# spacejam/loghisto

Hardware: NVIDIA H100
Metric: histogram ingest throughput (samples/s) (higher is better)
Workload: dtype f64

## Files before the change

### loghisto_b200/csrc/lh_api.cu

```cuda
#include "../../include/loghisto_b200.h"
#include "lh_kernels.cuh"

#include <algorithm>
#include <cmath>
#include <condition_variable>
#include <cstdio>
#include <cstring>
#include <mutex>
#include <new>
#include <string>
#include <vector>
#include <unistd.h>

using namespace lh;

namespace {

struct WriterEvent { cudaStream_t stream; cudaEvent_t ev; };

struct Buffer {
    unsigned long long *d_buckets = nullptr;
    unsigned long long *d_counters = nullptr;
    uint32_t *d_flags = nullptr;
    unsigned int *d_hot = nullptr;
    unsigned long long hot_pending = 0;
    cudaEvent_t cleared = nullptr;
    std::vector<WriterEvent> writers;
};

enum SlotState { SLOT_FREE = 0, SLOT_ACQUIRED = 1 , SLOT_INFLIGHT = 2,
                 SLOT_WAITED = 3 ,
                 SLOT_FILLING = 4  };
struct Slot {
    void *h = nullptr; void *d = nullptr;
    cudaEvent_t done = nullptr;
    cudaEvent_t copied = nullptr;
    int state = SLOT_FREE;
    uint64_t seq = 0;
};

struct K1Variant {
    const char *name;
    void (*launch)(int grid, size_t smem, cudaStream_t s, const double *v32, size_t nvec,
                   const double *head, int nhead, const double *tail, int ntail, unsigned long long *counts,
                   uint32_t *flag, const Prec &pc);
    const void *func;
    int threads;
    size_t smem_fixed;
    int blocks_per_sm;
    size_t smem;
};

template <int THREADS, int UNROLL, int MINB>
void launch_ldg(int grid, size_t smem, cudaStream_t s, const double *v32, size_t nvec, const double *head, int nhead,
                const double *tail, int ntail, unsigned long long *counts, uint32_t *flag, const Prec &pc) {
    k_ingest_single_ldg<THREADS, UNROLL, MINB><<<grid, THREADS, smem, s>>>(v32, nvec, head, nhead, tail, ntail, counts, flag, pc);
}
template <int CW, int STAGES, int STAGE_BYTES, int MINB, bool FOLD>
void launch_bulk(int grid, size_t smem, cudaStream_t s, const double *v32, size_t nvec, const double *head, int nhead,
                 const double *tail, int ntail, unsigned long long *counts, uint32_t *flag, const Prec &pc) {
    k_ingest_single_bulk<CW, STAGES, STAGE_BYTES, MINB, FOLD><<<grid, (CW + 1) * 32, smem, s>>>(v32, nvec, head, nhead, tail, ntail, counts, flag, pc);
}
void launch_probe(int grid, size_t, cudaStream_t s, const double *v32, size_t nvec, const double *head, int nhead,
                  const double *tail, int ntail, unsigned long long *counts, uint32_t *flag, const Prec &pc) {
    k_stream_probe<512, 4><<<grid, 512, 0, s>>>(v32, nvec, head, nhead, tail, ntail, counts, flag, pc);
}

#define LDG_VARIANT(T, U, M) \
    { "ldg_t" #T "_u" #U "_b" #M, launch_ldg<T, U, M>, (const void *)k_ingest_single_ldg<T, U, M>, T, 0, 0, 0 }
#define BULK_VARIANT(W, S, B, M, F) \
    { "bulk2_w" #W "_s" #S "_" #B "_b" #M "_sign" #F, launch_bulk<W, S, B, M, F != 0>, (const void *)k_ingest_single_bulk<W, S, B, M, F != 0>, (W + 1) * 32, \
      (size_t)S * B + (size_t)S * 16, 0, 0 }

K1Variant g_k1_variants[] = {
    BULK_VARIANT(16, 4, 32768, 1, 1),
    BULK_VARIANT(16, 3, 65536, 1, 1),
    BULK_VARIANT(8, 4, 16384, 2, 1),
    LDG_VARIANT(512, 2, 2),
    { "probe_read_only_t512_u4", launch_probe, (const void *)k_stream_probe<512, 4>, 512, 0, 0, 0 },
    BULK_VARIANT(16, 4, 32768, 1, 0),
    BULK_VARIANT(16, 3, 65536, 1, 0),
};
constexpr int kNumK1Variants = (int)(sizeof(g_k1_variants) / sizeof(g_k1_variants[0]));
constexpr int kDefaultK1Variant = 6;

Prec make_prec(uint32_t precision) {
    Prec pc{};
    const double P = (double)precision;
    const double c1 = P * 0.6931471805599453094172321;
    pc.precision = P;
    pc.a_int = (uint32_t)std::floor(c1);
    pc.c1 = (float)c1;
    pc.c2 = (float)(c1 - (double)pc.a_int);
    pc.kb = (float)(-1023.0 * (double)pc.c2);
    const float eps = 0.000244140625f * (precision > 100 ? (float)P / 100.0f : 1.0f);
    pc.thresh = 0.5f - eps;
    pc.win = (uint32_t)std::floor(P * 63.0 * 0.6931471805599453094172321 + 0.5) + 1u;
    pc.a4 = pc.a_int * 4u;
    pc.coff = 0u - 1023u * pc.a4 - (0x4B400000u << 2);
    pc.coff0 = 0u - 1023u * pc.a_int - 0x4B400000u;
    return pc;
}

constexpr int kMaxRanks = LH_MAX_RANKS;
constexpr int kCommWords = 2 * LH_MAX_RANKS;
constexpr uint32_t kPeerMagic = 0x4C485052u;

struct PeerWire {
    uint32_t magic, abi, H, C;
    uint32_t precision, device;
    int64_t pid;
    uint64_t ctx_id;
    uint64_t ptr_buckets[2], ptr_flags[2], ptr_counters[2], ptr_comm, ptr_red;
    cudaIpcMemHandle_t ipc_buckets[2], ipc_flags[2], ipc_counters[2], ipc_comm, ipc_red;
};
static_assert(sizeof(PeerWire) <= LH_PEER_HANDLE_BYTES, "lh_peer_handle too small");

struct PeerMap {
    unsigned long long *buckets[2] = {nullptr, nullptr};
    uint32_t *flags[2] = {nullptr, nullptr};
    unsigned long long *counters[2] = {nullptr, nullptr};
    unsigned long long *comm = nullptr;
    unsigned long long *red = nullptr;
    bool ipc = false;
};

}

struct lh_ctx {
    lh_config cfg{};
    int device = 0;
    int sm_count = 0;
    uint32_t H = 0, C = 0;
    Prec pc{};
    Buffer buf[2];
    int active = 0;
    bool frozen = false;
    bool nnz_valid = false;
    cudaStream_t ingest_stream = nullptr, snap_stream = nullptr, copy_stream = nullptr;
    double *d_decomp = nullptr;
    unsigned long long *d_dropped = nullptr;
    double *d_ps[3] = {nullptr, nullptr, nullptr};
    char *d_res[3] = {nullptr, nullptr, nullptr};
    char *h_res[3] = {nullptr, nullptr, nullptr};
    cudaEvent_t res_done[3] = {nullptr, nullptr, nullptr};
    uint32_t res_np[3] = {0, 0, 0};
    uint64_t res_ticket[2] = {0, 0};
    uint64_t next_ticket = 1;
    uint32_t *d_nnz = nullptr, *d_offsets = nullptr;
    short *d_x_keys = nullptr; unsigned long long *d_x_counts = nullptr; size_t x_cap = 0;
    uint32_t *h_offsets = nullptr;
    short *h_x_keys = nullptr; unsigned long long *h_x_counts = nullptr; size_t hx_cap = 0;
    unsigned long long *h_counter_deltas = nullptr;
    std::vector<Slot> slots;
    uint64_t slot_seq = 0;
    size_t staging_bytes = 0;
    unsigned long long last_margin[2] = {0, 0};
    int k1_variant = kDefaultK1Variant;
    int k1_grid_mult = 1;
    int k1_reserve_sms = 0;
    int keyed_blocks_per_sm = 8;
    uint32_t hot_replicas = 1;
    int keyed_mode = 0;
    int64_t kp_chunk = 256 << 20;
    uint32_t wc_pf_tiles = 1;
    uint32_t wc_flush_samples = 24576;
    int wc_spt = 6;
    unsigned short *d_kp_queues = nullptr;
    unsigned int *d_kp_cnt = nullptr;
    uint4 *d_kp_rare = nullptr;
    size_t kp_cap = 0;
    int kp_parts = 0;
    const char *keyed_kernel = "";
    uint32_t comm_rank = 0, comm_world = 0;
    unsigned long long *d_comm = nullptr;
    unsigned int *d_comm_aux = nullptr;
    PeerMap peers[kMaxRanks];
    unsigned long long *d_red_buckets = nullptr;
    uint32_t *d_red_flags = nullptr;
    unsigned long long *d_red_counters = nullptr;
    bool view_reduced = false;
    bool view_counters_reduced = false;
    uint64_t comm_seq = 0;
    bool comm_two_shot = false;
    static constexpr int kCommRing = 8;
    cudaEvent_t comm_t0[kCommRing] = {}, comm_t1[kCommRing] = {};
    uint64_t ctx_id = 0;
    std::mutex rs_mu;
    cudaStream_t rs_stream = nullptr;
    unsigned long long *d_rs_rows = nullptr;
    uint32_t *d_rs_flags = nullptr, *d_rs_nnz = nullptr;
    bool rs_dirty = false;
    K1Variant k1[kNumK1Variants];
    static constexpr int kTimingRing = 16;
    cudaEvent_t ev_t0s[kTimingRing] = {}, ev_t1s[kTimingRing] = {};
    cudaEvent_t ev_t0 = nullptr, ev_t1 = nullptr;
    uint64_t ingest_seq = 0;
    bool timing_valid = false;
    lh_stats stats{};
    std::mutex mu;
    std::condition_variable slot_cv;
    std::string last_error;
};

namespace {

lh_status fail(lh_ctx *ctx, lh_status st, const char *what, cudaError_t e = cudaSuccess) {
    if (ctx) {
        char buf[512];
        if (e != cudaSuccess) snprintf(buf, sizeof buf, "%s: %s (%s)", what, cudaGetErrorName(e), cudaGetErrorString(e));
        else snprintf(buf, sizeof buf, "%s", what);
        ctx->last_error = buf;
    }
    return st;
}

#define LH_CUDA(ctx, call)                                                      \
    do {                                                                        \
        cudaError_t _e = (call);                                                \
        if (_e != cudaSuccess) return fail((ctx), LH_ERR_CUDA, #call, _e);      \
    } while (0)

lh_status before_write(lh_ctx *ctx, int b, cudaStream_t s) {
    LH_CUDA(ctx, cudaStreamWaitEvent(s, ctx->buf[b].cleared, 0));
    return LH_OK;
}
lh_status after_write(lh_ctx *ctx, int b, cudaStream_t s) {
    for (auto &w : ctx->buf[b].writers)
        if (w.stream == s) { LH_CUDA(ctx, cudaEventRecord(w.ev, s)); return LH_OK; }
    WriterEvent w{s, nullptr};
    LH_CUDA(ctx, cudaEventCreateWithFlags(&w.ev, cudaEventDisableTiming));
    LH_CUDA(ctx, cudaEventRecord(w.ev, s));
    ctx->buf[b].writers.push_back(w);
    return LH_OK;
}

void next_timing_slot(lh_ctx *ctx) {
    const int i = (int)(ctx->ingest_seq % lh_ctx::kTimingRing);
    ctx->ev_t0 = ctx->ev_t0s[i];
    ctx->ev_t1 = ctx->ev_t1s[i];
    ctx->ingest_seq++;
}

cudaStream_t pick_stream(lh_ctx *ctx, void *stream) { return stream ? (cudaStream_t)stream : ctx->ingest_stream; }

int grid_1d(lh_ctx *ctx, size_t n, int threads, int per_thread, int blocks_per_sm) {
    size_t need = (n + (size_t)threads * per_thread - 1) / ((size_t)threads * per_thread);
    size_t cap = (size_t)ctx->sm_count * blocks_per_sm;
    return (int)std::max<size_t>(1, std::min(need, cap));
}

lh_status launch_single(lh_ctx *ctx, uint32_t hid, const double *d_values, size_t n, cudaStream_t s) {
    if (hid >= ctx->H) return fail(ctx, LH_ERR_RANGE, "histogram_id >= max_histograms");
    if (((uintptr_t)d_values & 7u) != 0) return fail(ctx, LH_ERR_INVALID, "d_values must be 8-byte aligned");
    const int b = ctx->active;
    lh_status st = before_write(ctx, b, s);
    if (st != LH_OK) return st;
    unsigned long long *counts = ctx->buf[b].d_buckets + (size_t)hid * 65536u;
    uint32_t *flag = ctx->buf[b].d_flags + hid;
    const K1Variant &kv = ctx->k1[ctx->k1_variant];
    const int grid = std::max(1, ctx->sm_count - ctx->k1_reserve_sms) * kv.blocks_per_sm * ctx->k1_grid_mult;
    const size_t kMaxPerLaunch = std::min((size_t)1 << 36, (size_t)grid << 31);
    size_t done = 0;
    next_timing_slot(ctx);
    LH_CUDA(ctx, cudaEventRecord(ctx->ev_t0, s));
    while (done < n) {
        size_t m = std::min(n - done, kMaxPerLaunch);
        const double *p = d_values + done;
        int nhead = (int)(((32u - ((uintptr_t)p & 31u)) & 31u) / 8u);
        if ((size_t)nhead > m) nhead = (int)m;
        const double *head = p;
        const double *body = p + nhead;
        size_t nvec = (m - nhead) >> 2;
        const double *tail = body + nvec * 4;
        int ntail = (int)(m - nhead - nvec * 4);
        kv.launch(grid, kv.smem, s, body, nvec, head, nhead, tail, ntail, counts, flag, ctx->pc);
        LH_CUDA(ctx, cudaGetLastError());
        ctx->stats.kernel_launches++;
        done += m;
    }
    LH_CUDA(ctx, cudaEventRecord(ctx->ev_t1, s));
    ctx->timing_valid = true;
    ctx->stats.samples += n;
    return after_write(ctx, b, s);
}

lh_status fold_hot(lh_ctx *ctx, int b, cudaStream_t s) {
    const size_t cells = (size_t)ctx->H * 2u * ctx->pc.win;
    int grid = (int)std::min<size_t>((cells + 255) / 256, (size_t)ctx->sm_count * 16);
    k_fold_hot<<<grid, 256, 0, s>>>(ctx->buf[b].d_hot, ctx->buf[b].d_buckets, ctx->buf[b].d_flags, cells, ctx->hot_replicas, ctx->pc.win);
    LH_CUDA(ctx, cudaGetLastError());
    ctx->stats.kernel_launches++;
    ctx->buf[b].hot_pending = 0;
    return LH_OK;
}

KeyedOut keyed_out(lh_ctx *ctx, int b) {
    KeyedOut o{};
    o.hot = ctx->buf[b].d_hot; o.buckets = ctx->buf[b].d_buckets; o.flags = ctx->buf[b].d_flags;
    o.dropped = ctx->d_dropped; o.H = ctx->H;
    return o;
}

uint32_t ks_ids_per_pass(const lh_ctx *ctx) { return std::max<uint32_t>(1, (uint32_t)(KS_SMEM_BYTES / ((size_t)ctx->pc.win * 4))); }

constexpr size_t kSmemBudget = 227 * 1024;
template <typename IdT, typename ValT, int SPT>
lh_status launch_keyed_wc_spt(lh_ctx *ctx, int b, const IdT *ids, const ValT *vals, size_t n4x4, cudaStream_t s, bool *used, size_t *taken,
                              const IdT *ids2 = nullptr, const long long *vals2 = nullptr, size_t n2 = 0, size_t *taken2 = nullptr) {
    *used = false;
    *taken = 0;
    if (taken2) *taken2 = 0;
    const int P = std::min(ctx->sm_count - ctx->k1_reserve_sms, (int)WC_MAX_PARTS);
    if (P < 8 || n4x4 + n2 == 0) return LH_OK;
    const uint32_t ids_per = (ctx->H + P - 1) / P;
    using S = WcShape<SPT>;
    const size_t hist_bytes = (((size_t)ids_per * ctx->pc.win + 3) & ~(size_t)3) * 4;
    uint32_t row_cap = 0;
    size_t smem = 0;
    for (uint32_t cap_try : {256u, 192u, 128u}) {
        smem = hist_bytes + 2 * WC_MAX_PARTS * 4 + (size_t)(P + 1) * (cap_try + WC_ROW_EXTRA) * 2;
        if (smem <= kSmemBudget) { row_cap = cap_try; break; }
    }
    if (!row_cap || (size_t)ids_per * ctx->pc.win > 65535) return LH_OK;
    if (ctx->keyed_mode != 2 && n4x4 + n2 < ((size_t)1 << 22)) return LH_OK;
    n4x4 = n4x4 / S::TILE * S::TILE;
    n2 = n2 / S::TILE * S::TILE;
    if (n4x4 + n2 == 0) return LH_OK;
    const size_t slice_max = std::max<size_t>(1, ((size_t)ctx->kp_chunk + (size_t)P * S::TILE - 1) / ((size_t)P * S::TILE));
    const size_t tiles_all = n4x4 / S::TILE + n2 / S::TILE;
    const size_t nchunks = (tiles_all + slice_max * P - 1) / (slice_max * P);
    const size_t slice_tiles = std::max<size_t>(1, (tiles_all + nchunks * P - 1) / (nchunks * P));
    const size_t expect = slice_max * S::TILE / P;
    const size_t cap = ((expect * 5 / 4 + 3 * WC_LINE + WC_LINE - 1) / WC_LINE) * WC_LINE;
    if (!ctx->d_kp_queues || ctx->kp_cap != cap || ctx->kp_parts != P) {
        cudaFree(ctx->d_kp_queues); cudaFree(ctx->d_kp_cnt); cudaFree(ctx->d_kp_rare);
        ctx->d_kp_queues = nullptr; ctx->d_kp_cnt = nullptr; ctx->d_kp_rare = nullptr;
        LH_CUDA(ctx, cudaMalloc(&ctx->d_kp_rare, (size_t)P * WC_RARE_CAP * sizeof(uint4)));
        LH_CUDA(ctx, cudaMalloc(&ctx->d_kp_queues, (size_t)2 * P * P * cap * sizeof(unsigned short)));
        LH_CUDA(ctx, cudaMalloc(&ctx->d_kp_cnt, ((size_t)2 * P * P + 1) * sizeof(unsigned int)));
        ctx->kp_cap = cap; ctx->kp_parts = P;
    }
    const void *fn = (const void *)k_ingest_keyed_wc<IdT, ValT, SPT, false>;
    if constexpr (std::is_same<ValT, double>::value) {
        if (n2) fn = (const void *)k_ingest_keyed_wc<IdT, double, SPT, true>;
    }
    LH_CUDA(ctx, cudaFuncSetAttribute(fn, cudaFuncAttributeMaxDynamicSharedMemorySize, (int)smem));
    unsigned int *d_barrier = ctx->d_kp_cnt + (size_t)2 * P * P;
    LH_CUDA(ctx, cudaMemsetAsync(d_barrier, 0, sizeof(unsigned int), s));
    WcParams prm{};
    prm.ids = ids; prm.vals = vals; prm.n = n4x4; prm.ids_per = ids_per; prm.cap = (uint32_t)cap;
    prm.ids2 = ids2; prm.vals2 = vals2; prm.n2 = n2;
    prm.inv_p = (uint32_t)(((uint64_t)1 << 32) / (uint64_t)P) + 1u;
    const double room = (double)row_cap - 63.0;
    const double m_max = std::pow((-3.5 + std::sqrt(3.5 * 3.5 + 4.0 * room)) / 2.0, 2.0);
    const uint32_t flush_samples = std::min<uint32_t>(ctx->wc_flush_samples, (uint32_t)(m_max * P));
    prm.flush_tiles = std::max<uint32_t>(1u, flush_samples / S::TILE);
    prm.pf_tiles = ctx->wc_pf_tiles;
    prm.row_cap = row_cap;
    prm.row_stride = row_cap + WC_ROW_EXTRA;
    prm.slice_tiles = (uint32_t)slice_tiles; prm.queues = ctx->d_kp_queues; prm.q_cnt = ctx->d_kp_cnt;
    prm.barrier = d_barrier; prm.rare = ctx->d_kp_rare; prm.o = keyed_out(ctx, b);
    Prec pc = ctx->pc;
    void *args[] = {&prm, &pc};
    LH_CUDA(ctx, cudaLaunchCooperativeKernel(fn, dim3(P), dim3(S::THREADS), args, smem, s));
    ctx->stats.kernel_launches++;
    *used = true;
    *taken = n4x4;
    if (taken2) *taken2 = n2;
    return LH_OK;
}
template <typename IdT, typename ValT>
lh_status launch_keyed_wc(lh_ctx *ctx, int b, const IdT *ids, const ValT *vals, size_t n4x4, cudaStream_t s, bool *used, size_t *taken,
                          const IdT *ids2 = nullptr, const long long *vals2 = nullptr, size_t n2 = 0, size_t *taken2 = nullptr) {
#define LH_WC_SHAPE(code) case code: return launch_keyed_wc_spt<IdT, ValT, code>(ctx, b, ids, vals, n4x4, s, used, taken, ids2, vals2, n2, taken2);
    switch (ctx->wc_spt) {
        LH_WC_SHAPE(6) LH_WC_SHAPE(4) LH_WC_SHAPE(3)
        default: return launch_keyed_wc_spt<IdT, ValT, 8>(ctx, b, ids, vals, n4x4, s, used, taken, ids2, vals2, n2, taken2);
    }
#undef LH_WC_SHAPE
}

template <typename IdT, typename ValT>
lh_status launch_keyed(lh_ctx *ctx, const IdT *d_ids, const ValT *d_vals, size_t n, cudaStream_t s) {
    if (((uintptr_t)d_vals & 7u) || ((uintptr_t)d_ids & (sizeof(IdT) - 1)))
        return fail(ctx, LH_ERR_INVALID, "ids / values are not naturally aligned");
    const int b = ctx->active;
    lh_status st = before_write(ctx, b, s);
    if (st != LH_OK) return st;
    constexpr int T = 256;
    const KeyedOut ko = keyed_out(ctx, b);
    next_timing_slot(ctx);
    LH_CUDA(ctx, cudaEventRecord(ctx->ev_t0, s));
    size_t done = 0;
    while (done < n) {
        const unsigned long long kCap = 0xFFFFFFFFull;
        if (ctx->buf[b].hot_pending >= kCap - (1ull << 30)) { st = fold_hot(ctx, b, s); if (st != LH_OK) return st; }
        size_t m = (size_t)std::min<unsigned long long>(n - done, kCap - ctx->buf[b].hot_pending);
        const IdT *ids = d_ids + done;
        const ValT *vals = d_vals + done;
        size_t head = std::min<size_t>(m, ((32u - ((uintptr_t)vals & 31u)) & 31u) / 8u);
        bool vec_ok = (((uintptr_t)(ids + head)) & (4 * sizeof(IdT) - 1)) == 0;
        size_t n4 = vec_ok ? (m - head) / 4 : 0;
        size_t tail_off = head + n4 * 4;
        if (!vec_ok) { head = 0; tail_off = 0; }
        if (head) {
            k_ingest_keyed<IdT, ValT, T><<<1, T, 0, s>>>(ids, vals, head, ko, ctx->pc);
            ctx->stats.kernel_launches++;
        }
        size_t hot_used = 0;
        if (n4) {
            bool used = false;
            constexpr uint32_t KS_MAX_PASSES = 4;
            const uint32_t per_max = ks_ids_per_pass(ctx);
            const uint32_t passes = (ctx->H + per_max - 1) / per_max;
            if (passes <= KS_MAX_PASSES && ctx->keyed_mode == 0 && n4 >= 4096) {
                const uint32_t per = (ctx->H + passes - 1) / passes;
                const size_t smem = ((size_t)per * ctx->pc.win + 4) * 4;
                const void *fn = (const void *)k_ingest_keyed_small<IdT, ValT>;
                LH_CUDA(ctx, cudaFuncSetAttribute(fn, cudaFuncAttributeMaxDynamicSharedMemorySize, (int)smem));
                int grid = (int)std::max<size_t>(1, std::min<size_t>((size_t)(ctx->sm_count - ctx->k1_reserve_sms),
                                                                      n4 / (KS_THREADS * 16)));
                for (uint32_t lo = 0; lo < ctx->H; lo += per) {
                    const uint32_t cnt = std::min(per, ctx->H - lo);
                    k_ingest_keyed_small<IdT, ValT><<<grid, KS_THREADS, smem, s>>>(ids + head, vals + head, n4, lo, cnt, ko, ctx->pc);
                    ctx->stats.kernel_launches++;
                }
                used = true;
                hot_used = n4 * 4;
                ctx->keyed_kernel = "k_ingest_keyed_small";
            }
            if (!used && ctx->keyed_mode != 1) {
                size_t taken = 0;
                st = launch_keyed_wc<IdT, ValT>(ctx, b, ids + head, vals + head, n4 * 4, s, &used, &taken);
                if (st != LH_OK) return st;
                if (used) {
                    ctx->keyed_kernel = "k_ingest_keyed_wc";
                    tail_off = head + taken;
                }
            }
            if (!used) {
                int grid = grid_1d(ctx, n4, T, 1, ctx->keyed_blocks_per_sm);
                k_ingest_keyed_vec<IdT, ValT, T><<<grid, T, 0, s>>>(ids + head, vals + head, n4, ctx->hot_replicas, ko, ctx->pc);
                ctx->stats.kernel_launches++;
                hot_used = n4 * 4;
                ctx->keyed_kernel = "k_ingest_keyed_vec";
            }
        }
        if (tail_off < m) {
            size_t r = m - tail_off;
            int grid = grid_1d(ctx, r, T, 1, ctx->keyed_blocks_per_sm);
            k_ingest_keyed<IdT, ValT, T><<<grid, T, 0, s>>>(ids + tail_off, vals + tail_off, r, ko, ctx->pc);
            ctx->stats.kernel_launches++;
        }
        LH_CUDA(ctx, cudaGetLastError());
        ctx->buf[b].hot_pending += hot_used;
        done += m;
    }
    LH_CUDA(ctx, cudaEventRecord(ctx->ev_t1, s));
    ctx->timing_valid = true;
    ctx->stats.samples += n;
    return after_write(ctx, b, s);
}

template <typename IdT>
lh_status launch_keyed_pair(lh_ctx *ctx, const IdT *ids_f, const double *vals_f, size_t n_f, const IdT *ids_ns, const long long *vals_ns,
                            size_t n_ns, cudaStream_t s) {
    auto aligned = [](const void *v, const void *i) { return (((uintptr_t)v & 31u) == 0) && (((uintptr_t)i & (4 * sizeof(IdT) - 1)) == 0); };
    const uint32_t small_passes = (ctx->H + ks_ids_per_pass(ctx) - 1) / ks_ids_per_pass(ctx);
    const bool small = small_passes <= 4 && ctx->keyed_mode == 0;
    const bool fuse = n_f && n_ns && ctx->keyed_mode != 1 && !small && aligned(vals_f, ids_f) && aligned(vals_ns, ids_ns);
    if (fuse) {
        const int b = ctx->active;
        lh_status st = before_write(ctx, b, s);
        if (st != LH_OK) return st;
        next_timing_slot(ctx);
        LH_CUDA(ctx, cudaEventRecord(ctx->ev_t0, s));
        bool used = false;
        size_t took_f = 0, took_ns = 0;
        st = launch_keyed_wc<IdT, double>(ctx, b, ids_f, vals_f, n_f, s, &used, &took_f, ids_ns, vals_ns, n_ns, &took_ns);
        if (st != LH_OK) return st;
        if (used) {
            constexpr int T = 256;
            const KeyedOut ko = keyed_out(ctx, b);
            ctx->keyed_kernel = "k_ingest_keyed_wc";
            if (took_f < n_f) {
                k_ingest_keyed<IdT, double, T><<<grid_1d(ctx, n_f - took_f, T, 1, ctx->keyed_blocks_per_sm), T, 0, s>>>(
                    ids_f + took_f, vals_f + took_f, n_f - took_f, ko, ctx->pc);
                ctx->stats.kernel_launches++;
            }
            if (took_ns < n_ns) {
                k_ingest_keyed<IdT, long long, T><<<grid_1d(ctx, n_ns - took_ns, T, 1, ctx->keyed_blocks_per_sm), T, 0, s>>>(
                    ids_ns + took_ns, vals_ns + took_ns, n_ns - took_ns, ko, ctx->pc);
                ctx->stats.kernel_launches++;
            }
            LH_CUDA(ctx, cudaGetLastError());
            LH_CUDA(ctx, cudaEventRecord(ctx->ev_t1, s));
            ctx->timing_valid = true;
            ctx->stats.samples += n_f + n_ns;
            return after_write(ctx, b, s);
        }
        st = after_write(ctx, b, s);
        if (st != LH_OK) return st;
    }
    lh_status st = n_f ? launch_keyed<IdT, double>(ctx, ids_f, vals_f, n_f, s) : LH_OK;
    if (st != LH_OK) return st;
    return n_ns ? launch_keyed<IdT, long long>(ctx, ids_ns, vals_ns, n_ns, s) : LH_OK;
}

template <typename IdT>
lh_status launch_counter(lh_ctx *ctx, const IdT *d_ids, const uint64_t *d_amounts, size_t n, cudaStream_t s) {
    const int b = ctx->active;
    lh_status st = before_write(ctx, b, s);
    if (st != LH_OK) return st;
    next_timing_slot(ctx);
    LH_CUDA(ctx, cudaEventRecord(ctx->ev_t0, s));
    if (n) {
        constexpr int T = 512;
        const unsigned long long *amts = reinterpret_cast<const unsigned long long *>(d_amounts);
        if (ctx->C <= (uint32_t)K2_SMEM_COUNTERS) {
            size_t head = std::min<size_t>(n, ((32u - ((uintptr_t)amts & 31u)) & 31u) / 8u);
            const bool vec_ok = (((uintptr_t)(d_ids + head)) & (4 * sizeof(IdT) - 1)) == 0 && (((uintptr_t)amts & 7u) == 0);
            size_t n4 = vec_ok ? (n - head) / 4 : 0;
            if (n4 < 4096) { head = 0; n4 = 0; }
            const size_t tail_off = head + n4 * 4;
            if (head) {
                k_counter_add_smem<IdT, T><<<1, T, (size_t)ctx->C * 8, s>>>(d_ids, amts, head, ctx->buf[b].d_counters, ctx->C, ctx->d_dropped);
                ctx->stats.kernel_launches++;
            }
            if (n4) {
                const int grid = (int)std::max<size_t>(1, std::min<size_t>((size_t)std::max(1, ctx->sm_count - ctx->k1_reserve_sms) * 2, n4 / (T * 4)));
                k_counter_add_smem_vec<IdT, T><<<grid, T, (size_t)ctx->C * 8, s>>>(d_ids + head, amts + head, n4, ctx->buf[b].d_counters, ctx->C, ctx->d_dropped);
                ctx->stats.kernel_launches++;
            }
            if (tail_off < n) {
                int grid = grid_1d(ctx, n - tail_off, T, 8, 2);
                k_counter_add_smem<IdT, T><<<grid, T, (size_t)ctx->C * 8, s>>>(d_ids + tail_off, amts + tail_off, n - tail_off, ctx->buf[b].d_counters, ctx->C, ctx->d_dropped);
                ctx->stats.kernel_launches++;
            }
        } else {
            int grid = grid_1d(ctx, n, T, 4, 4);
            k_counter_add<IdT, T><<<grid, T, 0, s>>>(d_ids, amts, n, ctx->buf[b].d_counters, ctx->C, ctx->d_dropped);
            ctx->stats.kernel_launches++;
        }
        LH_CUDA(ctx, cudaGetLastError());
    }
    LH_CUDA(ctx, cudaEventRecord(ctx->ev_t1, s));
    ctx->timing_valid = true;
    ctx->stats.counter_ops += n;
    return after_write(ctx, b, s);
}

lh_status slot_wait_free(lh_ctx *ctx, std::unique_lock<std::mutex> &lk, int *out) {
    for (;;) {
        int best = -1, fresh = -1, waited = 0;
        for (size_t i = 0; i < ctx->slots.size(); i++) {
            if (ctx->slots[i].state == SLOT_WAITED || ctx->slots[i].state == SLOT_FILLING) waited++;
            if (ctx->slots[i].state != SLOT_FREE) continue;
            if (ctx->slots[i].h) { *out = (int)i; return LH_OK; }
            if (fresh < 0) fresh = (int)i;
        }
        for (size_t i = 0; i < ctx->slots.size(); i++)
            if (ctx->slots[i].state == SLOT_INFLIGHT && cudaEventQuery(ctx->slots[i].done) == cudaSuccess) {
                ctx->slots[i].state = SLOT_FREE;
                *out = (int)i;
                return LH_OK;
            }
        cudaGetLastError();
        if (fresh >= 0) {
            Slot &sl = ctx->slots[fresh];
            cudaError_t e = cudaMallocHost(&sl.h, ctx->staging_bytes);
            if (e == cudaSuccess) e = cudaMalloc(&sl.d, ctx->staging_bytes);
            if (e != cudaSuccess) {
                if (sl.h) cudaFreeHost(sl.h);
                sl.h = nullptr; sl.d = nullptr;
                return fail(ctx, e == cudaErrorMemoryAllocation ? LH_ERR_NOMEM : LH_ERR_CUDA, "allocating a staging slot", e);
            }
            *out = fresh;
            return LH_OK;
        }
        for (size_t i = 0; i < ctx->slots.size(); i++)
            if (ctx->slots[i].state == SLOT_INFLIGHT && (best < 0 || ctx->slots[i].seq < ctx->slots[best].seq)) best = (int)i;
        if (best >= 0) {
            ctx->slots[best].state = SLOT_WAITED;
            cudaEvent_t ev = ctx->slots[best].done;
            lk.unlock();
            cudaError_t e = cudaEventSynchronize(ev);
            lk.lock();
            ctx->slots[best].state = SLOT_FREE;
            ctx->slot_cv.notify_all();
            if (e != cudaSuccess) return fail(ctx, LH_ERR_CUDA, "cudaEventSynchronize(slot)", e);
            *out = best;
            return LH_OK;
        }
        if (!waited) return fail(ctx, LH_ERR_STATE, "every staging slot is acquired and none is in flight");
        ctx->slot_cv.wait(lk);
    }
}

void comm_unmap(lh_ctx *ctx) {
    for (int r = 0; r < kMaxRanks; r++) {
        PeerMap &pm = ctx->peers[r];
        if (pm.ipc) {
            for (int b = 0; b < 2; b++) {
                if (pm.buckets[b]) cudaIpcCloseMemHandle(pm.buckets[b]);
                if (pm.flags[b]) cudaIpcCloseMemHandle(pm.flags[b]);
                if (pm.counters[b]) cudaIpcCloseMemHandle(pm.counters[b]);
            }
            if (pm.comm) cudaIpcCloseMemHandle(pm.comm);
            if (pm.red) cudaIpcCloseMemHandle(pm.red);
        }
        pm = PeerMap{};
    }
    ctx->comm_world = 0;
}

lh_status comm_alloc_reduced(lh_ctx *ctx) {
    if (ctx->d_red_buckets) return LH_OK;
    const size_t bucket_bytes = (size_t)ctx->H * 65536u * 8u;
    LH_CUDA(ctx, cudaMalloc(&ctx->d_red_buckets, bucket_bytes));
    LH_CUDA(ctx, cudaMalloc(&ctx->d_red_flags, (size_t)ctx->H * 4));
    LH_CUDA(ctx, cudaMalloc(&ctx->d_red_counters, (size_t)ctx->C * 8));
    LH_CUDA(ctx, cudaMemsetAsync(ctx->d_red_buckets, 0, bucket_bytes, ctx->snap_stream));
    LH_CUDA(ctx, cudaMemsetAsync(ctx->d_red_flags, 0, (size_t)ctx->H * 4, ctx->snap_stream));
    LH_CUDA(ctx, cudaMemsetAsync(ctx->d_red_counters, 0, (size_t)ctx->C * 8, ctx->snap_stream));
    LH_CUDA(ctx, cudaStreamSynchronize(ctx->snap_stream));
    return LH_OK;
}

bool is_pinned_or_managed(const void *p) {
    cudaPointerAttributes a;
    if (cudaPointerGetAttributes(&a, p) != cudaSuccess) { cudaGetLastError(); return false; }
    return a.type == cudaMemoryTypeHost || a.type == cudaMemoryTypeManaged;
}

}

extern "C" uint32_t lh_abi_version(void) { return LH_ABI_VERSION; }

extern "C" const char *lh_strerror(lh_status st) {
    switch (st) {
    case LH_OK: return "ok";
    case LH_ERR_INVALID: return "invalid argument";
    case LH_ERR_CUDA: return "CUDA runtime error";
    case LH_ERR_NOMEM: return "out of memory";
    case LH_ERR_NO_DEVICE: return "no usable CUDA device (there is no CPU fallback)";
    case LH_ERR_STATE: return "call out of order";
    case LH_ERR_RANGE: return "id or size out of range";
    default: return "unknown status";
    }
}

extern "C" const char *lh_last_error(const lh_ctx *ctx) { return ctx ? ctx->last_error.c_str() : ""; }

extern "C" lh_status lh_create(const lh_config *cfg, lh_ctx **out) {
    if (!cfg || !out || cfg->struct_size != sizeof(lh_config) || cfg->max_histograms == 0 || cfg->max_counters == 0)
        return LH_ERR_INVALID;
    if (cfg->precision > LH_MAX_PRECISION) return LH_ERR_RANGE;
    *out = nullptr;
    int ndev = 0;
    if (cudaGetDeviceCount(&ndev) != cudaSuccess || ndev == 0) { cudaGetLastError(); return LH_ERR_NO_DEVICE; }
    if (cfg->device < 0 || cfg->device >= ndev) return LH_ERR_NO_DEVICE;
    lh_ctx *ctx = new (std::nothrow) lh_ctx();
    if (!ctx) return LH_ERR_NOMEM;
    ctx->cfg = *cfg;
    ctx->device = cfg->device;
    ctx->H = cfg->max_histograms;
    ctx->C = cfg->max_counters;
    ctx->pc = make_prec(cfg->precision ? cfg->precision : 100);
    {
        static std::mutex id_mu;
        static uint64_t next_id = 1;
        std::lock_guard<std::mutex> lk(id_mu);
        ctx->ctx_id = next_id++;
    }
    {
        const size_t one = (size_t)ctx->H * 2u * ctx->pc.win * 4u;
        ctx->hot_replicas = (uint32_t)std::max<size_t>(1, std::min<size_t>(32, ((size_t)20 << 20) / one));
    }
    ctx->staging_bytes = cfg->staging_bytes ? (size_t)cfg->staging_bytes : ((size_t)32 << 20);
    ctx->staging_bytes = (ctx->staging_bytes + 255) & ~(size_t)255;
    const uint32_t nslots = cfg->staging_slots ? cfg->staging_slots : 3;

#define LH_CREATE_CUDA(call)                                                            \
    do {                                                                                \
        cudaError_t _e = (call);                                                        \
        if (_e != cudaSuccess) {                                                        \
            fprintf(stderr, "loghisto_b200: lh_create: %s failed: %s\n", #call, cudaGetErrorString(_e)); \
            lh_destroy(ctx);                                                            \
            return _e == cudaErrorMemoryAllocation ? LH_ERR_NOMEM : LH_ERR_CUDA;        \
        }                                                                               \
    } while (0)

    LH_CREATE_CUDA(cudaSetDevice(ctx->device));
    cudaDeviceProp prop;
    LH_CREATE_CUDA(cudaGetDeviceProperties(&prop, ctx->device));
    if (prop.major != 9 || prop.minor != 0) {
        fprintf(stderr, "loghisto_b200: device %d is sm_%d%d; this library is built for sm_90a only\n", ctx->device, prop.major, prop.minor);
        lh_destroy(ctx);
        return LH_ERR_NO_DEVICE;
    }
    ctx->sm_count = prop.multiProcessorCount;
    LH_CREATE_CUDA(cudaStreamCreateWithFlags(&ctx->ingest_stream, cudaStreamNonBlocking));
    LH_CREATE_CUDA(cudaStreamCreateWithFlags(&ctx->copy_stream, cudaStreamNonBlocking));
    {
        int least = 0, greatest = 0;
        LH_CREATE_CUDA(cudaDeviceGetStreamPriorityRange(&least, &greatest));
        LH_CREATE_CUDA(cudaStreamCreateWithPriority(&ctx->snap_stream, cudaStreamNonBlocking, greatest));
    }
    for (int i = 0; i < lh_ctx::kTimingRing; i++) {
        LH_CREATE_CUDA(cudaEventCreate(&ctx->ev_t0s[i]));
        LH_CREATE_CUDA(cudaEventCreate(&ctx->ev_t1s[i]));
    }
    for (int i = 0; i < lh_ctx::kCommRing; i++) {
        LH_CREATE_CUDA(cudaEventCreate(&ctx->comm_t0[i]));
        LH_CREATE_CUDA(cudaEventCreate(&ctx->comm_t1[i]));
    }

    const size_t bucket_bytes = (size_t)ctx->H * 65536u * 8u, counter_bytes = (size_t)ctx->C * 8u;
    const size_t hot_bytes = (size_t)ctx->hot_replicas * ctx->H * 2u * ctx->pc.win * 4u;
    for (int b = 0; b < 2; b++) {
        LH_CREATE_CUDA(cudaMalloc(&ctx->buf[b].d_buckets, bucket_bytes));
        LH_CREATE_CUDA(cudaMalloc(&ctx->buf[b].d_counters, counter_bytes));
        LH_CREATE_CUDA(cudaMalloc(&ctx->buf[b].d_flags, (size_t)ctx->H * 4u));
        LH_CREATE_CUDA(cudaMemsetAsync(ctx->buf[b].d_buckets, 0, bucket_bytes, ctx->snap_stream));
        LH_CREATE_CUDA(cudaMemsetAsync(ctx->buf[b].d_counters, 0, counter_bytes, ctx->snap_stream));
        LH_CREATE_CUDA(cudaMemsetAsync(ctx->buf[b].d_flags, 0, (size_t)ctx->H * 4u, ctx->snap_stream));
        LH_CREATE_CUDA(cudaMalloc(&ctx->buf[b].d_hot, hot_bytes));
        LH_CREATE_CUDA(cudaMemsetAsync(ctx->buf[b].d_hot, 0, hot_bytes, ctx->snap_stream));
        LH_CREATE_CUDA(cudaEventCreateWithFlags(&ctx->buf[b].cleared, cudaEventDisableTiming));
        LH_CREATE_CUDA(cudaEventRecord(ctx->buf[b].cleared, ctx->snap_stream));
    }
    LH_CREATE_CUDA(cudaMalloc(&ctx->d_decomp, 65536 * sizeof(double)));
    k_fill_decompress<<<65536 / 256, 256, 0, ctx->snap_stream>>>(ctx->d_decomp, ctx->pc.precision);
    LH_CREATE_CUDA(cudaGetLastError());
    LH_CREATE_CUDA(cudaMalloc(&ctx->d_comm, kCommWords * 8));
    LH_CREATE_CUDA(cudaMemsetAsync(ctx->d_comm, 0, kCommWords * 8, ctx->snap_stream));
    LH_CREATE_CUDA(cudaMalloc(&ctx->d_comm_aux, 16));
    LH_CREATE_CUDA(cudaMemsetAsync(ctx->d_comm_aux, 0, 16, ctx->snap_stream));
    LH_CREATE_CUDA(cudaMalloc(&ctx->d_dropped, 8));
    LH_CREATE_CUDA(cudaMemsetAsync(ctx->d_dropped, 0, 8, ctx->snap_stream));
    for (int i = 0; i < 3; i++) {
        const size_t res_bytes = (size_t)ctx->H * (24 + LH_MAX_PERCENTILES * 12);
        LH_CREATE_CUDA(cudaMalloc(&ctx->d_ps[i], LH_MAX_PERCENTILES * sizeof(double)));
        LH_CREATE_CUDA(cudaMalloc(&ctx->d_res[i], res_bytes));
        LH_CREATE_CUDA(cudaMallocHost(&ctx->h_res[i], res_bytes));
        LH_CREATE_CUDA(cudaEventCreateWithFlags(&ctx->res_done[i], cudaEventDisableTiming));
    }
    LH_CREATE_CUDA(cudaMalloc(&ctx->d_nnz, (size_t)ctx->H * 4));
    LH_CREATE_CUDA(cudaMalloc(&ctx->d_offsets, ((size_t)ctx->H + 1) * 4));
    LH_CREATE_CUDA(cudaMallocHost(&ctx->h_offsets, ((size_t)ctx->H + 1) * 4));
    LH_CREATE_CUDA(cudaMallocHost(&ctx->h_counter_deltas, counter_bytes));

    ctx->slots.resize(nslots);
    for (auto &sl : ctx->slots) {
        LH_CREATE_CUDA(cudaEventCreateWithFlags(&sl.done, cudaEventDisableTiming));
        LH_CREATE_CUDA(cudaEventCreateWithFlags(&sl.copied, cudaEventDisableTiming));
    }

    LH_CREATE_CUDA(cudaFuncSetAttribute((const void *)k_reduce, cudaFuncAttributeMaxDynamicSharedMemorySize, 100 * 1024));
    LH_CREATE_CUDA(cudaFuncSetAttribute((const void *)k_peer_allreduce, cudaFuncAttributeMaxDynamicSharedMemorySize, 64 * 1024));
    LH_CREATE_CUDA(cudaFuncSetAttribute((const void *)k_counter_add_smem<unsigned short, 512>, cudaFuncAttributeMaxDynamicSharedMemorySize, K2_SMEM_COUNTERS * 8));
    LH_CREATE_CUDA(cudaFuncSetAttribute((const void *)k_counter_add_smem<unsigned int, 512>, cudaFuncAttributeMaxDynamicSharedMemorySize, K2_SMEM_COUNTERS * 8));
    LH_CREATE_CUDA(cudaFuncSetAttribute((const void *)k_counter_add_smem_vec<unsigned short, 512>, cudaFuncAttributeMaxDynamicSharedMemorySize, K2_SMEM_COUNTERS * 8));
    LH_CREATE_CUDA(cudaFuncSetAttribute((const void *)k_counter_add_smem_vec<unsigned int, 512>, cudaFuncAttributeMaxDynamicSharedMemorySize, K2_SMEM_COUNTERS * 8));
    for (int i = 0; i < kNumK1Variants; i++) {
        ctx->k1[i] = g_k1_variants[i];
        const bool probe = ctx->k1[i].launch == launch_probe;
        const size_t hist = ((size_t)2 * ctx->pc.win + 8) * 4;
        ctx->k1[i].smem = probe ? 0 : ctx->k1[i].smem_fixed + hist;
        if (ctx->k1[i].smem > kSmemBudget) {
// ... 637 lines not shown
    w.precision = (uint32_t)ctx->pc.precision; w.device = (uint32_t)ctx->device;
    w.pid = (int64_t)getpid(); w.ctx_id = ctx->ctx_id;
    for (int b = 0; b < 2; b++) {
        w.ptr_buckets[b] = (uint64_t)(uintptr_t)ctx->buf[b].d_buckets;
        w.ptr_flags[b] = (uint64_t)(uintptr_t)ctx->buf[b].d_flags;
        w.ptr_counters[b] = (uint64_t)(uintptr_t)ctx->buf[b].d_counters;
        LH_CUDA(ctx, cudaIpcGetMemHandle(&w.ipc_buckets[b], ctx->buf[b].d_buckets));
        LH_CUDA(ctx, cudaIpcGetMemHandle(&w.ipc_flags[b], ctx->buf[b].d_flags));
        LH_CUDA(ctx, cudaIpcGetMemHandle(&w.ipc_counters[b], ctx->buf[b].d_counters));
    }
    w.ptr_comm = (uint64_t)(uintptr_t)ctx->d_comm;
    LH_CUDA(ctx, cudaIpcGetMemHandle(&w.ipc_comm, ctx->d_comm));
    if (lh_status st = comm_alloc_reduced(ctx)) return st;
    w.ptr_red = (uint64_t)(uintptr_t)ctx->d_red_buckets;
    LH_CUDA(ctx, cudaIpcGetMemHandle(&w.ipc_red, ctx->d_red_buckets));
    memset(out, 0, sizeof *out);
    memcpy(out->bytes, &w, sizeof w);
    return LH_OK;
}

extern "C" lh_status lh_comm_import(lh_ctx *ctx, uint32_t rank, uint32_t world, const lh_peer_handle *all) {
    LH_ENTER(ctx);
    if (!all || world < 1 || world > (uint32_t)kMaxRanks || rank >= world) return fail(ctx, LH_ERR_INVALID, "bad rank / world / handles");
    if (ctx->frozen) return fail(ctx, LH_ERR_STATE, "lh_comm_import during a snapshot");
    comm_unmap(ctx);
    const int64_t my_pid = (int64_t)getpid();
    for (uint32_t r = 0; r < world; r++) {
        PeerWire w;
        memcpy(&w, all[r].bytes, sizeof w);
        if (w.magic != kPeerMagic || w.abi != LH_ABI_VERSION) return fail(ctx, LH_ERR_INVALID, "peer handle is not from this library version");
        if (w.H != ctx->H || w.C != ctx->C || w.precision != (uint32_t)ctx->pc.precision)
            return fail(ctx, LH_ERR_INVALID, "peer context has a different shape (max_histograms / max_counters / precision)");
        PeerMap &pm = ctx->peers[r];
        if (r == rank) {
            if (w.ctx_id != ctx->ctx_id || w.pid != my_pid) return fail(ctx, LH_ERR_INVALID, "handles[rank] is not this context's own handle");
            for (int b = 0; b < 2; b++) { pm.buckets[b] = ctx->buf[b].d_buckets; pm.flags[b] = ctx->buf[b].d_flags; pm.counters[b] = ctx->buf[b].d_counters; }
            pm.comm = ctx->d_comm;
            if (lh_status st = comm_alloc_reduced(ctx)) return st;
            pm.red = ctx->d_red_buckets;
            continue;
        }
        if (w.pid == my_pid) {
            if ((int)w.device != ctx->device) {
                int can = 0;
                LH_CUDA(ctx, cudaDeviceCanAccessPeer(&can, ctx->device, (int)w.device));
                if (!can) return fail(ctx, LH_ERR_NO_DEVICE, "no peer access between the two devices");
                cudaError_t e = cudaDeviceEnablePeerAccess((int)w.device, 0);
                if (e != cudaSuccess && e != cudaErrorPeerAccessAlreadyEnabled) return fail(ctx, LH_ERR_CUDA, "cudaDeviceEnablePeerAccess", e);
                cudaGetLastError();
            }
            for (int b = 0; b < 2; b++) {
                pm.buckets[b] = (unsigned long long *)(uintptr_t)w.ptr_buckets[b];
                pm.flags[b] = (uint32_t *)(uintptr_t)w.ptr_flags[b];
                pm.counters[b] = (unsigned long long *)(uintptr_t)w.ptr_counters[b];
            }
            pm.comm = (unsigned long long *)(uintptr_t)w.ptr_comm;
            pm.red = (unsigned long long *)(uintptr_t)w.ptr_red;
        } else {
            pm.ipc = true;
            for (int b = 0; b < 2; b++) {
                LH_CUDA(ctx, cudaIpcOpenMemHandle((void **)&pm.buckets[b], w.ipc_buckets[b], cudaIpcMemLazyEnablePeerAccess));
                LH_CUDA(ctx, cudaIpcOpenMemHandle((void **)&pm.flags[b], w.ipc_flags[b], cudaIpcMemLazyEnablePeerAccess));
                LH_CUDA(ctx, cudaIpcOpenMemHandle((void **)&pm.counters[b], w.ipc_counters[b], cudaIpcMemLazyEnablePeerAccess));
            }
            LH_CUDA(ctx, cudaIpcOpenMemHandle((void **)&pm.comm, w.ipc_comm, cudaIpcMemLazyEnablePeerAccess));
            LH_CUDA(ctx, cudaIpcOpenMemHandle((void **)&pm.red, w.ipc_red, cudaIpcMemLazyEnablePeerAccess));
        }
    }
    ctx->comm_rank = rank;
    ctx->comm_world = world;
    return LH_OK;
}

extern "C" lh_status lh_snapshot_allreduce(lh_ctx *ctx, uint32_t include_counters, uint64_t *seq_out) {
    LH_ENTER(ctx);
    if (!ctx->frozen) return fail(ctx, LH_ERR_STATE, "no snapshot in progress");
    if (ctx->comm_world < 2) return fail(ctx, LH_ERR_STATE, "lh_comm_import has not been called with world >= 2");
    if (ctx->view_reduced) return fail(ctx, LH_ERR_STATE, "this snapshot has already been all-reduced");
    const int f = ctx->active ^ 1;
    cudaStream_t s = ctx->snap_stream;
    PeerParams p{};
    p.rank = ctx->comm_rank; p.world = ctx->comm_world; p.H = ctx->H; p.C = ctx->C; p.win = ctx->pc.win;
    p.do_counters = include_counters ? 1u : 0u; p.frozen = (uint32_t)f;
    p.seq = ++ctx->comm_seq;
    p.timeout_ns = 10ull * 1000ull * 1000ull * 1000ull;
    for (uint32_t r = 0; r < ctx->comm_world; r++) {
        p.buckets[r] = ctx->peers[r].buckets[f];
        p.flags[r] = ctx->peers[r].flags[f];
        p.counters[r] = ctx->peers[r].counters[f];
        p.comm[r] = ctx->peers[r].comm;
    }
    p.out_buckets = ctx->d_red_buckets; p.out_flags = ctx->d_red_flags; p.out_counters = ctx->d_red_counters;
    p.block_counter = ctx->d_comm_aux; p.status = ctx->d_comm_aux + 1;
    p.cells = reinterpret_cast<unsigned long long *>(ctx->d_comm_aux + 2);
    for (uint32_t r = 0; r < ctx->comm_world; r++) p.out_peer[r] = ctx->peers[r].red;
    const size_t payload = (size_t)ctx->H * (2u * ctx->pc.win - 1u) * 8u;
    p.two_shot = payload >= (1u << 20) ? 1u : 0u;
    ctx->comm_two_shot = p.two_shot != 0;
    const int ring = (int)(p.seq % lh_ctx::kCommRing);
    const size_t items = (size_t)ctx->H * (65536u / K5_CHUNK);
    int grid = (int)std::min<size_t>(items, ctx->H == 1 ? 5 : 16);
    LH_CUDA(ctx, cudaEventRecord(ctx->comm_t0[ring], s));
    if (p.two_shot) {
        PeerParams pa = p;
        pa.arrive_only = 1;
        k_peer_allreduce<<<1, K5_THREADS, ctx->H, s>>>(pa);
        LH_CUDA(ctx, cudaGetLastError());
        ctx->stats.kernel_launches++;
        grid = (int)std::min<size_t>((ctx->H + ctx->comm_world - 1) / ctx->comm_world, (size_t)std::max(1, std::min(128, ctx->sm_count - 20)));
    }
    k_peer_allreduce<<<grid, K5_THREADS, ctx->H, s>>>(p);
    LH_CUDA(ctx, cudaGetLastError());
    LH_CUDA(ctx, cudaEventRecord(ctx->comm_t1[ring], s));
    ctx->stats.kernel_launches++;
    ctx->view_reduced = true;
    ctx->view_counters_reduced = include_counters != 0;
    ctx->nnz_valid = false;
    if (seq_out) *seq_out = p.seq;
    return LH_OK;
}

extern "C" lh_status lh_comm_allreduce_ms(lh_ctx *ctx, uint64_t seq, float *ms) {
    if (!ctx || !ms) return LH_ERR_INVALID;
    cudaEvent_t e0, e1;
    {
        std::lock_guard<std::mutex> lk(ctx->mu);
        if (seq == 0 || seq > ctx->comm_seq || ctx->comm_seq - seq >= (uint64_t)lh_ctx::kCommRing)
            return fail(ctx, LH_ERR_STATE, "that all-reduce is unknown or its events were recycled");
        const int ring = (int)(seq % lh_ctx::kCommRing);
        e0 = ctx->comm_t0[ring]; e1 = ctx->comm_t1[ring];
    }
    cudaError_t e = cudaEventSynchronize(e1);
    if (e == cudaSuccess) e = cudaEventElapsedTime(ms, e0, e1);
    std::lock_guard<std::mutex> lk(ctx->mu);
    if (e != cudaSuccess) return fail(ctx, LH_ERR_CUDA, "lh_comm_allreduce_ms", e);
    return LH_OK;
}

extern "C" lh_status lh_comm_info(lh_ctx *ctx, lh_comm_stats *out) {
    LH_ENTER(ctx);
    if (!out) return fail(ctx, LH_ERR_INVALID, "out is NULL");
    memset(out, 0, sizeof *out);
    out->rank = ctx->comm_rank; out->world = ctx->comm_world; out->allreduces = ctx->comm_seq;
    if (ctx->comm_world >= 2) {
        unsigned int aux[2] = {0, 0};
        LH_CUDA(ctx, cudaMemcpy(aux, ctx->d_comm_aux, 8, cudaMemcpyDeviceToHost));
        out->status = aux[1];
        unsigned long long cells = 0;
        LH_CUDA(ctx, cudaMemcpy(&cells, ctx->d_comm_aux + 2, 8, cudaMemcpyDeviceToHost));
        out->last_bytes_from_peers = ctx->comm_two_shot ? cells * 8u * (ctx->comm_world - 1) / ctx->comm_world : cells * 8u * (ctx->comm_world - 1);
    }
    return LH_OK;
}

extern "C" const char *lh_keyed_kernel_name(lh_ctx *ctx) { return ctx ? ctx->keyed_kernel : ""; }

extern "C" lh_status lh_compress_f64(lh_ctx *ctx, const double *d_values, size_t n, int16_t *d_out, int mode, void *stream) {
    LH_ENTER(ctx);
    if (n && (!d_values || !d_out)) return fail(ctx, LH_ERR_INVALID, "NULL input");
    if (!n) return LH_OK;
    cudaStream_t s = pick_stream(ctx, stream);
    k_compress_probe<<<(unsigned)((n + 255) / 256), 256, 0, s>>>(d_values, n, d_out, mode, ctx->pc);
    LH_CUDA(ctx, cudaGetLastError());
    return LH_OK;
}

extern "C" lh_status lh_decompress_table(lh_ctx *ctx, double *h_out) {
    LH_ENTER(ctx);
    if (!h_out) return fail(ctx, LH_ERR_INVALID, "h_out is NULL");
    LH_CUDA(ctx, cudaMemcpy(h_out, ctx->d_decomp, 65536 * sizeof(double), cudaMemcpyDeviceToHost));
    return LH_OK;
}

extern "C" lh_status lh_fastpath_margin(lh_ctx *ctx, const double *d_values, size_t n, double *h_max_err, uint64_t *h_n_slow, void *stream) {
    LH_ENTER(ctx);
    if (n && !d_values) return fail(ctx, LH_ERR_INVALID, "NULL input");
    cudaStream_t s = pick_stream(ctx, stream);
    unsigned long long *d = nullptr;
    LH_CUDA(ctx, cudaMalloc(&d, 24));
    LH_CUDA(ctx, cudaMemsetAsync(d, 0, 24, s));
    if (n) k_fastpath_margin<<<(unsigned)((n + 255) / 256), 256, 0, s>>>(d_values, n, d, ctx->pc);
    unsigned long long h[3];
    cudaError_t e = cudaMemcpyAsync(h, d, 24, cudaMemcpyDeviceToHost, s);
    if (e == cudaSuccess) e = cudaStreamSynchronize(s);
    cudaFree(d);
    if (e != cudaSuccess) return fail(ctx, LH_ERR_CUDA, "lh_fastpath_margin", e);
    const unsigned long long worst = std::max(h[0], h[2]);
    if (h_max_err) memcpy(h_max_err, &worst, 8);
    if (h_n_slow) *h_n_slow = h[1];
    ctx->last_margin[0] = h[0]; ctx->last_margin[1] = h[2];
    return LH_OK;
}

extern "C" lh_status lh_fastpath_margin_detail(lh_ctx *ctx, double *h_err_estimator1, double *h_err_estimator2) {
    LH_ENTER(ctx);
    if (h_err_estimator1) memcpy(h_err_estimator1, &ctx->last_margin[0], 8);
    if (h_err_estimator2) memcpy(h_err_estimator2, &ctx->last_margin[1], 8);
    return LH_OK;
}

extern "C" lh_status lh_gen_stream_f64(lh_ctx *ctx, int kind, uint64_t seed, uint64_t start, size_t n, double *d_out, void *stream) {
    LH_ENTER(ctx);
    if (n && !d_out) return fail(ctx, LH_ERR_INVALID, "d_out is NULL");
    if (!n) return LH_OK;
    k_gen_stream<<<ctx->sm_count * 8, 256, 0, pick_stream(ctx, stream)>>>(kind, seed, start, n, d_out);
    LH_CUDA(ctx, cudaGetLastError());
    return LH_OK;
}
extern "C" lh_status lh_gen_ids_u16(lh_ctx *ctx, int kind, uint64_t seed, uint64_t start, size_t n, uint32_t n_ids, uint16_t *d_out, void *stream) {
    LH_ENTER(ctx);
    if (n && !d_out) return fail(ctx, LH_ERR_INVALID, "d_out is NULL");
    if (n_ids == 0 || n_ids > 65536) return fail(ctx, LH_ERR_RANGE, "n_ids must be in 1..65536");
    if (!n) return LH_OK;
    k_gen_ids_u16<<<ctx->sm_count * 8, 256, 0, pick_stream(ctx, stream)>>>(kind, seed, start, n, n_ids, d_out);
    LH_CUDA(ctx, cudaGetLastError());
    return LH_OK;
}

extern "C" lh_status lh_get_stats(lh_ctx *ctx, lh_stats *out) {
    LH_ENTER(ctx);
    if (!out) return fail(ctx, LH_ERR_INVALID, "out is NULL");
    unsigned long long dropped = 0;
    LH_CUDA(ctx, cudaMemcpy(&dropped, ctx->d_dropped, 8, cudaMemcpyDeviceToHost));
    ctx->stats.dropped = dropped;
    *out = ctx->stats;
    return LH_OK;
}
extern "C" lh_status lh_sync(lh_ctx *ctx) {
    LH_ENTER(ctx);
    std::vector<cudaStream_t> streams = {ctx->ingest_stream, ctx->copy_stream, ctx->snap_stream};
    for (int b = 0; b < 2; b++)
        for (auto &w : ctx->buf[b].writers)
            if (std::find(streams.begin(), streams.end(), w.stream) == streams.end()) streams.push_back(w.stream);
    _lk.unlock();
    cudaError_t e = cudaSuccess;
    for (cudaStream_t st : streams) { cudaError_t x = cudaStreamSynchronize(st); if (e == cudaSuccess) e = x; }
    _lk.lock();
    if (e != cudaSuccess) return fail(ctx, LH_ERR_CUDA, "lh_sync", e);
    for (auto &sl : ctx->slots)
        if (sl.state == SLOT_INFLIGHT && cudaEventQuery(sl.done) == cudaSuccess) sl.state = SLOT_FREE;
    cudaGetLastError();
    return LH_OK;
}
extern "C" void *lh_ingest_stream(lh_ctx *ctx) { return ctx ? (void *)ctx->ingest_stream : nullptr; }

extern "C" lh_status lh_device_alloc(lh_ctx *ctx, size_t bytes, void **d_out) {
    LH_ENTER(ctx);
    if (!d_out) return fail(ctx, LH_ERR_INVALID, "d_out is NULL");
    cudaError_t e = cudaMalloc(d_out, bytes ? bytes : 1);
    if (e != cudaSuccess) return fail(ctx, e == cudaErrorMemoryAllocation ? LH_ERR_NOMEM : LH_ERR_CUDA, "cudaMalloc", e);
    return LH_OK;
}
extern "C" lh_status lh_device_free(lh_ctx *ctx, void *d_ptr) {
    LH_ENTER(ctx);
    LH_CUDA(ctx, cudaFree(d_ptr));
    return LH_OK;
}
extern "C" lh_status lh_host_alloc_pinned(lh_ctx *ctx, size_t bytes, void **h_out) {
    LH_ENTER(ctx);
    if (!h_out) return fail(ctx, LH_ERR_INVALID, "h_out is NULL");
    cudaError_t e = cudaMallocHost(h_out, bytes ? bytes : 1);
    if (e != cudaSuccess) return fail(ctx, e == cudaErrorMemoryAllocation ? LH_ERR_NOMEM : LH_ERR_CUDA, "cudaMallocHost", e);
    return LH_OK;
}
extern "C" lh_status lh_host_free_pinned(lh_ctx *ctx, void *h_ptr) {
    LH_ENTER(ctx);
    LH_CUDA(ctx, cudaFreeHost(h_ptr));
    return LH_OK;
}
extern "C" lh_status lh_memcpy_h2d(lh_ctx *ctx, void *d_dst, const void *h_src, size_t bytes) {
    LH_ENTER(ctx);
    LH_CUDA(ctx, cudaMemcpy(d_dst, h_src, bytes, cudaMemcpyHostToDevice));
    return LH_OK;
}
extern "C" lh_status lh_memcpy_d2h(lh_ctx *ctx, void *h_dst, const void *d_src, size_t bytes) {
    LH_ENTER(ctx);
    LH_CUDA(ctx, cudaMemcpy(h_dst, d_src, bytes, cudaMemcpyDeviceToHost));
    return LH_OK;
}

extern "C" lh_status lh_tune(lh_ctx *ctx, const char *key, int64_t value) {
    LH_ENTER(ctx);
    if (!key) return fail(ctx, LH_ERR_INVALID, "key is NULL");
    if (!strcmp(key, "k1")) {
        if (value < 0 || value >= kNumK1Variants) return fail(ctx, LH_ERR_RANGE, "unknown k1 variant");
        ctx->k1_variant = (int)value;
        return LH_OK;
    }
    if (!strcmp(key, "k1_grid_mult")) {
        if (value < 1 || value > 64) return fail(ctx, LH_ERR_RANGE, "k1_grid_mult out of range");
        ctx->k1_grid_mult = (int)value;
        return LH_OK;
    }
    if (!strcmp(key, "k1_reserve_sms")) {
        if (value < 0 || value >= ctx->sm_count) return fail(ctx, LH_ERR_RANGE, "k1_reserve_sms out of range");
        ctx->k1_reserve_sms = (int)value;
        return LH_OK;
    }
    if (!strcmp(key, "keyed_mode")) {
        if (value < 0 || value > 2) return fail(ctx, LH_ERR_RANGE, "keyed_mode is 0 (auto), 1 (L2 atomics) or 2 (owner-partitioned, write-combining)");
        ctx->keyed_mode = (int)value;
        return LH_OK;
    }
    if (!strcmp(key, "wc_pf")) {
        if (value < 0 || value > 8) return fail(ctx, LH_ERR_RANGE, "wc_pf is 0 ... 8 tiles");
        ctx->wc_pf_tiles = (uint32_t)value;
        return LH_OK;
    }
    if (!strcmp(key, "wc_flush")) {
        if (value < 4096 || value > 65536) return fail(ctx, LH_ERR_RANGE, "wc_flush is 4096 ... 65536 samples");
        ctx->wc_flush_samples = (uint32_t)value;
        return LH_OK;
    }
    if (!strcmp(key, "wc_spt")) {
        if (value != 4 && value != 6 && value != 3 && value != 8)
            return fail(ctx, LH_ERR_RANGE, "wc_spt is a shape code: 6 (896 threads x 4 samples), 4 (1024 x 4), 3 (768 x 4) or 8 (512 x 8)");
        ctx->wc_spt = (int)value;
        return LH_OK;
    }
    if (!strcmp(key, "kp_chunk")) {
        if (value < (1 << 16) || value > ((int64_t)1 << 28)) return fail(ctx, LH_ERR_RANGE, "kp_chunk out of range");
        ctx->kp_chunk = value;
        return LH_OK;
    }
    if (!strcmp(key, "keyed_blocks_per_sm")) {
        if (value < 1 || value > 32) return fail(ctx, LH_ERR_RANGE, "keyed_blocks_per_sm out of range");
        ctx->keyed_blocks_per_sm = (int)value;
        return LH_OK;
    }
    return fail(ctx, LH_ERR_INVALID, "unknown tuning key");
}

extern "C" int32_t lh_k1_variant_count(void) { return kNumK1Variants; }
extern "C" int32_t lh_k1_variant_current(lh_ctx *ctx) { return ctx ? ctx->k1_variant : -1; }
extern "C" const char *lh_k1_variant_name(lh_ctx *ctx, int32_t i) {
    if (!ctx || i < 0 || i >= kNumK1Variants) return "";
    return ctx->k1[i].name;
}

extern "C" uint64_t lh_ingest_seq(lh_ctx *ctx) {
    if (!ctx) return 0;
    std::lock_guard<std::mutex> lk(ctx->mu);
    return ctx->ingest_seq;
}

extern "C" lh_status lh_kernel_ms(lh_ctx *ctx, uint64_t seq, float *ms) {
    LH_ENTER(ctx);
    if (!ms) return fail(ctx, LH_ERR_INVALID, "ms is NULL");
    if (seq == 0 || seq > ctx->ingest_seq || ctx->ingest_seq - seq >= (uint64_t)lh_ctx::kTimingRing)
        return fail(ctx, LH_ERR_STATE, "that ingest launch is unknown or its events were recycled");
    const int i = (int)((seq - 1) % lh_ctx::kTimingRing);
    LH_CUDA(ctx, cudaEventSynchronize(ctx->ev_t1s[i]));
    LH_CUDA(ctx, cudaEventElapsedTime(ms, ctx->ev_t0s[i], ctx->ev_t1s[i]));
    return LH_OK;
}

extern "C" lh_status lh_last_kernel_ms(lh_ctx *ctx, float *ms) {
    LH_ENTER(ctx);
    if (!ms) return fail(ctx, LH_ERR_INVALID, "ms is NULL");
    if (!ctx->timing_valid) return fail(ctx, LH_ERR_STATE, "no ingest kernel has been launched");
    LH_CUDA(ctx, cudaEventSynchronize(ctx->ev_t1));
    LH_CUDA(ctx, cudaEventElapsedTime(ms, ctx->ev_t0, ctx->ev_t1));
    return LH_OK;
}
```

### loghisto_b200/csrc/lh_kernels.cuh

```cuda
#pragma once
#include "../../include/loghisto_b200.h"
#include <type_traits>
#include "lh_device.cuh"

namespace lh {

struct f64x4 { double a, b, c, d; };
__device__ __forceinline__ uint64_t policy_evict_first() {
    uint64_t p;
    asm("createpolicy.fractional.L2::evict_first.b64 %0, 1.0;" : "=l"(p));
    return p;
}
__device__ __forceinline__ void ldg_stream_u64x4(const void *p, unsigned long long (&r)[4]) {
    const uint64_t pol = policy_evict_first();
    asm volatile("ld.global.nc.L1::no_allocate.L2::cache_hint.v2.b64 {%0, %1}, [%2], %3;"
                 : "=l"(r[0]), "=l"(r[1]) : "l"(p), "l"(pol));
    asm volatile("ld.global.nc.L1::no_allocate.L2::cache_hint.v2.b64 {%0, %1}, [%2], %3;"
                 : "=l"(r[2]), "=l"(r[3]) : "l"((const char *)p + 16), "l"(pol));
}
__device__ __forceinline__ f64x4 ldg_stream_f64x4(const void *p) {
    unsigned long long u[4];
    ldg_stream_u64x4(p, u);
    f64x4 r;
    r.a = __longlong_as_double((long long)u[0]); r.b = __longlong_as_double((long long)u[1]);
// ... 61 lines not shown
        const uint32_t c = hist[slot];
        if (c) { atomicAdd(&counts[slot_to_key16(slot, win)], (unsigned long long)c); any = 1; }
    }
    any = __syncthreads_or(any);
    if (any && tid == 0) mark(flag, 1u);
}

__device__ __forceinline__ uint32_t fixup_slot(double v, const Prec &pc, unsigned long long *__restrict__ counts,
                                               uint32_t *flag) {
    const uint32_t key = key16_of(v, pc);
    uint32_t slot = key16_to_slot(key, pc.win);
    if (slot == 0xFFFFFFFFu) { add_bucket_global(counts, flag, key, 1ull, pc.win); slot = 2u * pc.win; }
    return slot;
}

__device__ __forceinline__ void bucket_stragglers(const double *p, int n, const Prec &pc,
                                                  unsigned long long *__restrict__ counts, uint32_t *flag) {
    for (int i = 0; i < n; i++) add_bucket_global(counts, flag, key16_of(p[i], pc), 1ull, pc.win);
}

template <int NS>
__device__ __forceinline__ void bucket_samples(const double (&v)[NS], uint32_t *hist, const Prec &pc,
                                               unsigned long long *__restrict__ counts, uint32_t *flag) {
    uint32_t idx[NS];
    bool slow[NS];
    bool any = false;
#pragma unroll
    for (int i = 0; i < NS; i++) { fast_candidate(v[i], pc, idx[i], slow[i]); any |= slow[i]; }
    if (__any_sync(0xFFFFFFFFu, any)) {
#pragma unroll
        for (int i = 0; i < NS; i++) {
            if (slow[i]) {
                const uint32_t key = exact_key16(v[i], pc.precision);
                uint32_t slot = key16_to_slot(key, pc.win);
                if (slot == 0xFFFFFFFFu) { add_bucket_global(counts, flag, key, 1ull, pc.win); slot = 2u * pc.win; }
                idx[i] = slot;
            }
        }
    }
#pragma unroll
    for (int i = 0; i < NS; i++) atomicAdd(&hist[idx[i]], 1u);
}

template <int THREADS, int UNROLL, int MINB>
__global__ void __launch_bounds__(THREADS, MINB)
k_ingest_single_ldg(const double *__restrict__ vals32, size_t nvec, const double *head, int nhead,
                    const double *tail, int ntail, unsigned long long *__restrict__ counts, uint32_t *flag, Prec pc) {
    extern __shared__ __align__(16) uint32_t s_hist[];
    for (uint32_t i = threadIdx.x; i < subhist_words(pc.win); i += THREADS) s_hist[i] = 0;
    __syncthreads();
    const char *base = reinterpret_cast<const char *>(vals32);

    constexpr size_t TILE = (size_t)THREADS * UNROLL;
    const size_t ntiles = nvec / TILE;
    f64x4 cur[UNROLL], nxt[UNROLL];
    size_t tile = blockIdx.x;
    if (tile < ntiles) {
#pragma unroll
        for (int u = 0; u < UNROLL; u++) cur[u] = ldg_stream_f64x4(base + (tile * TILE + (size_t)u * THREADS + threadIdx.x) * 32);
    }
    while (tile < ntiles) {
        const size_t nt = tile + gridDim.x;
        if (nt < ntiles) {
#pragma unroll
            for (int u = 0; u < UNROLL; u++) nxt[u] = ldg_stream_f64x4(base + (nt * TILE + (size_t)u * THREADS + threadIdx.x) * 32);
        }
        double v[4 * UNROLL];
#pragma unroll
        for (int u = 0; u < UNROLL; u++) { v[4 * u] = cur[u].a; v[4 * u + 1] = cur[u].b; v[4 * u + 2] = cur[u].c; v[4 * u + 3] = cur[u].d; }
        bucket_samples<4 * UNROLL>(v, s_hist, pc, counts, flag);
#pragma unroll
        for (int u = 0; u < UNROLL; u++) cur[u] = nxt[u];
        tile = nt;
    }
    if (blockIdx.x == ntiles % gridDim.x) {
        for (size_t j = ntiles * TILE * 4 + threadIdx.x; j < nvec * 4; j += THREADS)
            atomicAdd(&s_hist[fixup_slot(vals32[j], pc, counts, flag)], 1u);
        if (threadIdx.x == 0) { bucket_stragglers(head, nhead, pc, counts, flag); bucket_stragglers(tail, ntail, pc, counts, flag); }
    }
    __syncthreads();
    flush_subhist(s_hist, threadIdx.x, THREADS, counts, flag, pc.win);
}

template <int NS, bool FOLD_SIGN, int SHIFT = 2>
__device__ __forceinline__ void bucket_offsets_v2(const double (&v)[NS], const Prec &pc, uint32_t one_bits,
                                                  uint32_t (&off)[NS], bool (&flag)[NS]) {
    static_assert(NS % 2 == 0, "pairs");
    constexpr float MAGIC = 12582912.0f;
    const uint32_t negoff = pc.win << SHIFT;
    const uint32_t am = SHIFT ? pc.a4 : pc.a_int, cm = SHIFT ? pc.coff : pc.coff0;
#pragma unroll
    for (int i = 0; i < NS; i += 2) {
        const double x0 = __dadd_rn(1.0, fabs(v[i])), x1 = __dadd_rn(1.0, fabs(v[i + 1]));
        const uint32_t h0 = (uint32_t)__double2hiint(x0), h1 = (uint32_t)__double2hiint(x1);
        const uint32_t t0 = __funnelshift_l((uint32_t)__double2loint(x0), h0, 3);
        const uint32_t t1 = __funnelshift_l((uint32_t)__double2loint(x1), h1, 3);
        uint32_t m0, m1;
        asm("lop3.b32 %0, %1, 0x007FFFFF, %2, 0xEA;" : "=r"(m0) : "r"(t0), "r"(one_bits));
        asm("lop3.b32 %0, %1, 0x007FFFFF, %2, 0xEA;" : "=r"(m1) : "r"(t1), "r"(one_bits));
        float2 lg;
        asm("lg2.approx.ftz.f32 %0, %1;" : "=f"(lg.x) : "f"(__uint_as_float(m0)));
        asm("lg2.approx.ftz.f32 %0, %1;" : "=f"(lg.y) : "f"(__uint_as_float(m1)));
        const uint32_t e0 = h0 >> 20, e1 = h1 >> 20;
        const float2 ef = make_float2(__uint2float_rn(e0), __uint2float_rn(e1));
        const float2 a = make_float2(__fmaf_rn(ef.x, pc.c2, pc.kb), __fmaf_rn(ef.y, pc.c2, pc.kb));
        const float2 w = make_float2(__fmaf_rn(lg.x, pc.c1, a.x), __fmaf_rn(lg.y, pc.c1, a.y));
        const float2 r = make_float2(__fadd_rn(w.x, MAGIC), __fadd_rn(w.y, MAGIC));
        const float2 s = make_float2(__fadd_rn(r.x, -MAGIC), __fadd_rn(r.y, -MAGIC));
        const float2 d = make_float2(__fmaf_rn(s.x, -1.0f, w.x), __fmaf_rn(s.y, -1.0f, w.y));
        if (FOLD_SIGN) {
            flag[i] = (fabsf(d.x) > pc.thresh) | (h0 >= 0x43E00000u);
            flag[i + 1] = (fabsf(d.y) > pc.thresh) | (h1 >= 0x43E00000u);
            const uint32_t n0 = (uint32_t)__double2hiint(v[i]) >> 31, n1 = (uint32_t)__double2hiint(v[i + 1]) >> 31;
            off[i] = e0 * am + (__float_as_uint(r.x) << SHIFT) + (n0 * negoff + cm);
            off[i + 1] = e1 * am + (__float_as_uint(r.y) << SHIFT) + (n1 * negoff + cm);
        } else {
            flag[i] = (fabsf(d.x) > pc.thresh) | ((uint32_t)__double2hiint(v[i]) >= 0x43E00000u);
            flag[i + 1] = (fabsf(d.y) > pc.thresh) | ((uint32_t)__double2hiint(v[i + 1]) >= 0x43E00000u);
            off[i] = e0 * am + (__float_as_uint(r.x) << SHIFT) + cm;
            off[i + 1] = e1 * am + (__float_as_uint(r.y) << SHIFT) + cm;
        }
    }
}

template <int NS, bool FOLD_SIGN>
__device__ __forceinline__ void bucket_samples_v2(const double (&v)[NS], uint32_t *hist, const Prec &pc, uint32_t one_bits,
                                                  unsigned long long *__restrict__ counts, uint32_t *gflag) {
    uint32_t off[NS];
    bool flag[NS];
    bucket_offsets_v2<NS, FOLD_SIGN>(v, pc, one_bits, off, flag);
    bool any = false;
#pragma unroll
    for (int i = 0; i < NS; i++) any |= flag[i];
    if (__any_sync(0xFFFFFFFFu, any)) {
#pragma unroll
        for (int i = 0; i < NS; i++)
            if (__any_sync(0xFFFFFFFFu, flag[i])) {
                if (flag[i]) off[i] = fixup_slot(v[i], pc, counts, gflag) * 4u;
            }
    }
#pragma unroll
    for (int i = 0; i < NS; i++) atomicAdd(reinterpret_cast<uint32_t *>(reinterpret_cast<char *>(hist) + off[i]), 1u);
}

template <int THREADS, int UNROLL>
__global__ void __launch_bounds__(THREADS, 2)
k_stream_probe(const double *__restrict__ vals32, size_t nvec, const double *, int, const double *, int,
               unsigned long long *__restrict__ counts, uint32_t *, Prec) {
    const char *base = reinterpret_cast<const char *>(vals32);
    constexpr size_t TILE = (size_t)THREADS * UNROLL;
    const size_t ntiles = nvec / TILE;
    unsigned long long acc = 0;
    for (size_t tile = blockIdx.x; tile < ntiles; tile += gridDim.x) {
        f64x4 v[UNROLL];
#pragma unroll
        for (int u = 0; u < UNROLL; u++) v[u] = ldg_stream_f64x4(base + (tile * TILE + (size_t)u * THREADS + threadIdx.x) * 32);
#pragma unroll
        for (int u = 0; u < UNROLL; u++)
            acc ^= f64_as_u64(v[u].a) ^ f64_as_u64(v[u].b) ^ f64_as_u64(v[u].c) ^ f64_as_u64(v[u].d);
    }
    if (acc == 0x123456789ABCDEFull) counts[65535] = acc;
}

template <int CW, int STAGES, int STAGE_BYTES, int MINB, bool FOLD_SIGN>
__global__ void __launch_bounds__((CW + 1) * 32, MINB)
k_ingest_single_bulk(const double *__restrict__ vals32, size_t nvec32, const double *head, int nhead,
                     const double *tail, int ntail, unsigned long long *__restrict__ counts, uint32_t *flag, Prec pc) {
    const double2 *vals16 = reinterpret_cast<const double2 *>(vals32);
    const size_t nvec = nvec32 * 2;
    constexpr int CT = CW * 32;
    constexpr int STAGE_VEC = STAGE_BYTES / 16;
    constexpr int PER_THREAD = STAGE_VEC / CT;
    static_assert(STAGE_VEC % CT == 0, "stage must divide evenly over consumer threads");
    extern __shared__ __align__(128) unsigned char s_raw[];
    double2 *s_data = reinterpret_cast<double2 *>(s_raw);
    uint64_t *full = reinterpret_cast<uint64_t *>(s_raw + (size_t)STAGES * STAGE_BYTES);
    uint64_t *empty = full + STAGES;
    uint32_t *s_hist = reinterpret_cast<uint32_t *>(empty + STAGES);

    const int tid = threadIdx.x;
    const int warp = tid >> 5;
    for (uint32_t i = tid; i < subhist_words(pc.win); i += (CW + 1) * 32) s_hist[i] = 0;
    if (tid == 0) {
        for (int s = 0; s < STAGES; s++) { mbar_init(&full[s], 1); mbar_init(&empty[s], CW); }
        asm volatile("fence.mbarrier_init.release.cluster;" ::: "memory");
    }
    __syncthreads();

    const size_t ntiles = (nvec + STAGE_VEC - 1) / STAGE_VEC;
    if (warp == CW) {
        if ((tid & 31) == 0) {
            const uint64_t pol = policy_evict_first();
            uint32_t it = 0;
            for (size_t tile = blockIdx.x; tile < ntiles; tile += gridDim.x, it++) {
                const int s = it % STAGES;
                mbar_wait(&empty[s], ((it / STAGES) & 1) ^ 1);
                size_t first = tile * (size_t)STAGE_VEC;
                size_t rem = nvec - first;
                uint32_t bytes = (uint32_t)((rem < (size_t)STAGE_VEC ? rem : (size_t)STAGE_VEC) * 16);
                mbar_expect_tx(&full[s], bytes);
                bulk_g2s(s_data + (size_t)s * STAGE_VEC, vals16 + first, bytes, &full[s], pol);
            }
        }
    } else {
        uint32_t one_bits;
        asm volatile("mov.b32 %0, 0x3F800000;" : "=r"(one_bits));
        uint32_t it = 0;
        for (size_t tile = blockIdx.x; tile < ntiles; tile += gridDim.x, it++) {
            const int s = it % STAGES;
            mbar_wait(&full[s], (it / STAGES) & 1);
            const double2 *st = s_data + (size_t)s * STAGE_VEC;
            size_t first = tile * (size_t)STAGE_VEC;
            size_t rem = nvec - first;
            if (rem >= (size_t)STAGE_VEC) {
                double v[2 * PER_THREAD];
#pragma unroll
                for (int u = 0; u < PER_THREAD; u++) {
                    double2 d = st[u * CT + tid];
                    v[2 * u] = d.x; v[2 * u + 1] = d.y;
                }
                __syncwarp();
                if ((tid & 31) == 0) mbar_arrive(&empty[s]);
#pragma unroll
                for (int q = 0; q < 2 * PER_THREAD; q += 4) {
                    const double v4[4] = {v[q], v[q + 1], v[q + 2], v[q + 3]};
                    bucket_samples_v2<4, FOLD_SIGN>(v4, s_hist, pc, one_bits, counts, flag);
                }
            } else {
                for (int j = tid; j < (int)rem; j += CT) {
                    double2 d = st[j];
                    atomicAdd(&s_hist[fixup_slot(d.x, pc, counts, flag)], 1u);
                    atomicAdd(&s_hist[fixup_slot(d.y, pc, counts, flag)], 1u);
                }
                __syncwarp();
                if ((tid & 31) == 0) mbar_arrive(&empty[s]);
            }
        }
        if (blockIdx.x == 0 && tid == 0) { bucket_stragglers(head, nhead, pc, counts, flag); bucket_stragglers(tail, ntail, pc, counts, flag); }
    }
    __syncthreads();
    flush_subhist(s_hist, tid, (CW + 1) * 32, counts, flag, pc.win);
}

template <typename T> __device__ __forceinline__ double sample_to_f64(T v);
template <> __device__ __forceinline__ double sample_to_f64<double>(double v) { return v; }
template <> __device__ __forceinline__ double sample_to_f64<long long>(long long v) { return __ll2double_rn(v); }

struct KeyedOut {
    unsigned int *hot;
    unsigned long long *buckets;
    uint32_t *flags;
    unsigned long long *dropped;
    uint32_t H;
};

template <typename ValT>
__device__ __forceinline__ void keyed_one(uint32_t id, ValT raw, const Prec &pc, const KeyedOut &o, unsigned int *hot, uint64_t pol) {
    if (id >= o.H) { atomicAdd(o.dropped, 1ull); return; }
    double v = sample_to_f64<ValT>(raw);
    uint32_t idx; bool slow;
    fast_candidate(v, pc, idx, slow);
    if (slow) {
        uint32_t key = exact_key16(v, pc.precision);
        idx = key16_to_slot(key, pc.win);
        if (idx == 0xFFFFFFFFu) { add_bucket_global(o.buckets + (size_t)id * 65536u, o.flags + id, key, 1ull, pc.win); return; }
    }
    red_add_u32_keep(&hot[(size_t)id * (2u * pc.win) + idx], 1u, pol);
}
template <typename ValT>
__device__ __forceinline__ void keyed_one_direct(uint32_t id, ValT raw, const Prec &pc, const KeyedOut &o) {
    if (id >= o.H) { atomicAdd(o.dropped, 1ull); return; }
    add_bucket_global(o.buckets + (size_t)id * 65536u, o.flags + id, key16_of(sample_to_f64<ValT>(raw), pc), 1ull, pc.win);
}

template <typename ValT>
__device__ __noinline__ void keyed_one_slow(uint32_t id, unsigned long long raw, Prec pc, KeyedOut o) {
    ValT r;
    memcpy(&r, &raw, 8);
    keyed_one_direct<ValT>(id, r, pc, o);
}

template <typename IdT>
__device__ __forceinline__ void load_ids4(const IdT *ids, size_t g, uint32_t (&id4)[4]) {
    if (sizeof(IdT) == 2) {
        unsigned int lo, hi;
        asm volatile("ld.global.nc.L1::no_allocate.v2.u32 {%0, %1}, [%2];" : "=r"(lo), "=r"(hi)
                     : "l"(reinterpret_cast<const char *>(ids) + g * 8));
        id4[0] = lo & 0xFFFFu; id4[1] = lo >> 16; id4[2] = hi & 0xFFFFu; id4[3] = hi >> 16;
    } else {
        asm volatile("ld.global.nc.L1::no_allocate.v4.u32 {%0, %1, %2, %3}, [%4];" : "=r"(id4[0]), "=r"(id4[1]), "=r"(id4[2]), "=r"(id4[3])
                     : "l"(reinterpret_cast<const char *>(ids) + g * 16));
    }
}
__device__ __forceinline__ void load_vals4(const void *vals, size_t g, unsigned long long (&raw)[4]) {
    ldg_stream_u64x4(reinterpret_cast<const char *>(vals) + g * 32, raw);
}

template <typename IdT> struct IdPack;
template <> struct IdPack<unsigned short> {
    unsigned int lo, hi;
    __device__ __forceinline__ void load(const unsigned short *ids, size_t g) {
        asm volatile("ld.global.nc.L1::no_allocate.v2.u32 {%0, %1}, [%2];" : "=r"(lo), "=r"(hi) : "l"(reinterpret_cast<const char *>(ids) + g * 8));
    }
    __device__ __forceinline__ uint32_t get(int j) const { const unsigned int w = j < 2 ? lo : hi; return (j & 1) ? (w >> 16) : (w & 0xFFFFu); }
};
template <> struct IdPack<unsigned int> {
    unsigned int w[4];
    __device__ __forceinline__ void load(const unsigned int *ids, size_t g) {
        asm volatile("ld.global.nc.L1::no_allocate.v4.u32 {%0, %1, %2, %3}, [%4];" : "=r"(w[0]), "=r"(w[1]), "=r"(w[2]), "=r"(w[3])
                     : "l"(reinterpret_cast<const char *>(ids) + g * 16));
    }
    __device__ __forceinline__ uint32_t get(int j) const { return w[j]; }
};

template <typename IdT, typename ValT, int THREADS>
__global__ void __launch_bounds__(THREADS)
k_ingest_keyed_vec(const IdT *__restrict__ ids, const ValT *__restrict__ vals, size_t n4, uint32_t replicas, KeyedOut o, Prec pc) {
    unsigned int *hot = o.hot + (size_t)(blockIdx.x % replicas) * o.H * (2u * pc.win);
    const uint64_t pol = policy_evict_last();
    const size_t stride = (size_t)gridDim.x * THREADS;
    for (size_t g = (size_t)blockIdx.x * THREADS + threadIdx.x; g < n4; g += stride) {
        unsigned long long raw[4];
        uint32_t id4[4];
        load_vals4(vals, g, raw);
        load_ids4<IdT>(ids, g, id4);
#pragma unroll
        for (int j = 0; j < 4; j++) {
            ValT r;
            memcpy(&r, &raw[j], 8);
            keyed_one<ValT>(id4[j], r, pc, o, hot, pol);
        }
    }
}

template <typename IdT, typename ValT, int THREADS>
__global__ void __launch_bounds__(THREADS)
k_ingest_keyed(const IdT *__restrict__ ids, const ValT *__restrict__ vals, size_t n, KeyedOut o, Prec pc) {
    const size_t stride = (size_t)gridDim.x * THREADS;
    for (size_t i = (size_t)blockIdx.x * THREADS + threadIdx.x; i < n; i += stride)
        keyed_one_direct<ValT>((uint32_t)ids[i], vals[i], pc, o);
}

constexpr int KS_THREADS = 1024;
constexpr int KS_SMEM_BYTES = 196608;

template <typename IdT, typename ValT>
__global__ void __launch_bounds__(KS_THREADS, 1)
k_ingest_keyed_small(const IdT *__restrict__ ids, const ValT *__restrict__ vals, size_t n4,
                     uint32_t id_lo, uint32_t id_cnt, KeyedOut o, Prec pc) {
    extern __shared__ __align__(16) uint32_t ks_hist[];
    const uint32_t row = pc.win;
    const uint32_t words = id_cnt * row;
    for (uint32_t i = threadIdx.x; i <= words; i += KS_THREADS) ks_hist[i] = 0;
    __syncthreads();
    const uint64_t pol = policy_evict_last();
    uint32_t one_bits;
    asm volatile("mov.b32 %0, 0x3F800000;" : "=r"(one_bits));
    const uint32_t trash_off = words * 4u;

    const size_t stride = (size_t)gridDim.x * KS_THREADS;
    size_t base = (size_t)blockIdx.x * KS_THREADS;
    unsigned long long cur[4] = {0, 0, 0, 0}, nxt[4] = {0, 0, 0, 0};
    uint32_t cur_id[4] = {0, 0, 0, 0}, nxt_id[4] = {0, 0, 0, 0};
    if (base + threadIdx.x < n4) { load_vals4(vals, base + threadIdx.x, cur); load_ids4<IdT>(ids, base + threadIdx.x, cur_id); }
    for (; base < n4; base += stride) {
        const bool valid = base + threadIdx.x < n4;
        const size_t gn = base + stride + threadIdx.x;
        if (gn < n4) { load_vals4(vals, gn, nxt); load_ids4<IdT>(ids, gn, nxt_id); }
        double v[4];
#pragma unroll
        for (int i = 0; i < 4; i++) { ValT r; memcpy(&r, &cur[i], 8); v[i] = sample_to_f64<ValT>(r); }
        uint32_t off[4];
        bool flag[4];
        bucket_offsets_v2<4, false>(v, pc, one_bits, off, flag);
        bool any = false;
#pragma unroll
        for (int i = 0; i < 4; i++) {
            const uint32_t l = cur_id[i] - id_lo;
            const bool mine = valid & (l < id_cnt);
            const bool bad = valid & (cur_id[i] >= o.H) & (id_lo == 0);
            flag[i] = (mine & flag[i]) | bad;
            off[i] = mine ? off[i] + l * (row * 4u) : trash_off;
            any |= flag[i];
        }
        if (__any_sync(0xFFFFFFFFu, any)) {
#pragma unroll
            for (int i = 0; i < 4; i++) {
                if (!flag[i]) continue;
                ValT rv;
                memcpy(&rv, &cur[i], 8);
                keyed_one<ValT>(cur_id[i], rv, pc, o, o.hot, pol);
                off[i] = trash_off;
            }
        }
#pragma unroll
        for (int i = 0; i < 4; i++) atomicAdd(reinterpret_cast<uint32_t *>(reinterpret_cast<char *>(ks_hist) + off[i]), 1u);
#pragma unroll
        for (int i = 0; i < 4; i++) { cur[i] = nxt[i]; cur_id[i] = nxt_id[i]; }
    }
    __syncthreads();
    for (uint32_t i = threadIdx.x; i < words; i += KS_THREADS) {
        const uint32_t c = ks_hist[i];
        if (!c) continue;
        const uint32_t lid = i / row, slot = i - lid * row;
        atomicAdd(&o.hot[(size_t)(id_lo + lid) * (2u * pc.win) + slot], c);
    }
}

constexpr int WC_MAX_PARTS = 160;
constexpr int WC_LINE = 64;

template <int SPT> struct WcShape {
    static constexpr int THREADS = SPT == 4 ? 1024 : SPT == 6 ? 896 : SPT == 3 ? 768 : 512;
    static constexpr int PER = SPT == 8 ? 8 : 4;
    static constexpr int TILE = THREADS * PER;
};
constexpr int WC_ROW_EXTRA = WC_LINE + 8;

struct WcParams {
    const void *ids;
    const void *vals;
    size_t n;
    const void *ids2;
    const void *vals2;
    size_t n2;
    uint32_t ids_per;
    uint32_t cap;
    uint32_t slice_tiles;
    uint32_t inv_p;
    uint32_t flush_tiles;
    uint32_t pf_tiles;
    uint32_t row_cap;
    uint32_t row_stride;
    unsigned short *queues;
    unsigned int *q_cnt;
    unsigned int *barrier;
    uint4 *rare;
    KeyedOut o;
};
constexpr uint32_t WC_RARE_CAP = 8192;

__device__ __forceinline__ void grid_barrier(unsigned int *bar, unsigned int target) {
    __syncthreads();
    if (threadIdx.x == 0) {
        __threadfence();
        atomicAdd(bar, 1u);
        unsigned int v;
        do {
            asm volatile("ld.acquire.gpu.global.u32 %0, [%1];" : "=r"(v) : "l"(bar) : "memory");
        } while (v < target);
    }
    __syncthreads();
}

__device__ __forceinline__ void wc_spill(uint32_t rec, uint32_t owner, uint32_t P, const Prec &pc, const KeyedOut &o) {
    const uint32_t lid = rec / pc.win, slot = rec - lid * pc.win, id = lid * P + owner;
    add_bucket_global(o.buckets + (size_t)id * 65536u, o.flags + id, slot, 1ull, pc.win);
}

template <typename IdT, typename ValT, int SPT, bool PAIR = false>
__global__ void __launch_bounds__(WcShape<SPT>::THREADS, 1)
k_ingest_keyed_wc(WcParams prm, Prec pc) {
    static_assert(!PAIR || std::is_same<ValT, double>::value, "the int64 segment rides on the float64 instantiation");
    using S = WcShape<SPT>;
    constexpr int WC_THREADS = S::THREADS;
    constexpr int GROUPS = S::PER / 4;
    extern __shared__ __align__(16) unsigned char wc_smem[];
    const uint32_t P = gridDim.x, p = blockIdx.x, tid = threadIdx.x;
    unsigned int *s_hist = reinterpret_cast<unsigned int *>(wc_smem);
    const uint32_t hist_words = prm.ids_per * pc.win;
    unsigned int *s_fill = s_hist + ((hist_words + 3u) & ~3u);
    unsigned int *s_off = s_fill + WC_MAX_PARTS;
    unsigned short *s_buf = reinterpret_cast<unsigned short *>(s_off + WC_MAX_PARTS);
    uint32_t fill_addr = smem_u32(s_fill);
    const uint32_t hist_addr = smem_u32(s_hist);
    asm volatile("mov.b32 %0, %0;" : "+r"(fill_addr));
    const uint32_t buf_addr = fill_addr + 2u * WC_MAX_PARTS * 4u;
    unsigned int *s_rare = s_fill + (WC_MAX_PARTS - 1);
    uint4 *rareq = prm.rare + (size_t)p * WC_RARE_CAP;
    uint32_t negP = 0u - P;
    asm volatile("mov.b32 %0, %0;" : "+r"(negP));

    for (uint32_t i = tid; i < hist_words; i += WC_THREADS) s_hist[i] = 0;
    if (tid < WC_MAX_PARTS) { s_fill[tid] = 0; s_off[tid] = 0; }
    uint32_t one_bits;
    asm volatile("mov.b32 %0, 0x3F800000;" : "=r"(one_bits));
    __syncthreads();

    const size_t tiles_seg0 = prm.n / S::TILE;
    const size_t tiles_total = tiles_seg0 + (PAIR ? prm.n2 / S::TILE : 0);
    const size_t chunk_tiles = (size_t)prm.slice_tiles * P;
    const size_t nchunks = (tiles_total + chunk_tiles - 1) / chunk_tiles;
    const IdT *ids = reinterpret_cast<const IdT *>(prm.ids);
    const unsigned int cap = prm.cap;
    const uint32_t row_cap = prm.row_cap, row_stride = prm.row_stride;


    unsigned long long cur[GROUPS][4], nxt[GROUPS][4];
    IdPack<IdT> cur_id[GROUPS], nxt_id[GROUPS];
    uint32_t since_flush = 0;
    const char *vptr = nullptr;
    const IdT *iptr = nullptr;
    const size_t pf_v = (size_t)prm.pf_tiles * S::TILE * 8, pf_i = (size_t)prm.pf_tiles * S::TILE;
    auto load_tile = [&](const char *vp, const IdT *ip, unsigned long long (&raw)[GROUPS][4], IdPack<IdT> (&idp)[GROUPS]) {
#pragma unroll
        for (int g = 0; g < GROUPS; g++) {
            load_vals4(vp, (size_t)g * WC_THREADS, raw[g]);
            idp[g].load(ip, (size_t)g * WC_THREADS);
        }
    };

    for (size_t c = 0; c < nchunks; c++) {
        const size_t par = c & 1;
        unsigned short *qset = prm.queues + par * (size_t)P * P * cap;
        unsigned int *cset = prm.q_cnt + par * (size_t)P * P;
        const bool last_chunk = c + 1 == nchunks;
        const size_t tile0 = c * chunk_tiles + (size_t)p * prm.slice_tiles;
        const uint32_t ntile_all = tile0 >= tiles_total ? 0u : (uint32_t)min((size_t)prm.slice_tiles, tiles_total - tile0);
        auto bin_tile = [&](unsigned long long (&raw)[GROUPS][4], IdPack<IdT> (&idp)[GROUPS], const bool as_i64) {
            if constexpr (PAIR) {
                if (as_i64) {
#pragma unroll
                    for (int g = 0; g < GROUPS; g++)
#pragma unroll
                        for (int j = 0; j < 4; j++) raw[g][j] = (unsigned long long)__double_as_longlong(__ll2double_rn((long long)raw[g][j]));
                }
            }
#pragma unroll
            for (int g = 0; g < GROUPS; g++) {
                double v[4];
#pragma unroll
                for (int j = 0; j < 4; j++) { ValT r; memcpy(&r, &raw[g][j], 8); v[j] = sample_to_f64<ValT>(r); }
                uint32_t idx[4];
                bool flag[4];
                bucket_offsets_v2<4, false, 0>(v, pc, one_bits, idx, flag);
                bool any = false;
#pragma unroll
                for (int j = 0; j < 4; j++) {
                    const uint32_t id = idp[g].get(j);
                    const uint32_t lid = __umulhi(id, prm.inv_p), owner = lid * negP + id;
                    const uint32_t rec = lid * pc.win + idx[j];
                    const bool rare = flag[j] | (id >= prm.o.H);
                    const uint32_t oe = rare ? P : owner;
                    uint32_t pos;
                    asm volatile("atom.shared.add.u32 %0, [%1], 1;" : "=r"(pos) : "r"(fill_addr + oe * 4u) : "memory");
                    flag[j] = rare | (pos >= row_cap);
                    if (!flag[j])
                        asm volatile("st.shared.u16 [%0], %1;" ::"r"(buf_addr + (oe * row_stride + pos) * 2u), "h"((unsigned short)rec) : "memory");
                    any |= flag[j];
                }
                if (__any_sync(0xFFFFFFFFu, any)) {
#pragma unroll
                    for (int j = 0; j < 4; j++)
                        if (flag[j]) {
                            const unsigned int at = atomicAdd(s_rare, 1u);
                            if (at < WC_RARE_CAP) rareq[at] = make_uint4((unsigned int)raw[g][j], (unsigned int)(raw[g][j] >> 32), idp[g].get(j), 0u);
                            else keyed_one_slow<ValT>(idp[g].get(j), raw[g][j], pc, prm.o);
                        }
                }
            }
            if (++since_flush == prm.flush_tiles) {
                since_flush = 0;
                __syncthreads();
                constexpr uint32_t GROUPS_PER_WARP = 8;
                const uint32_t sub = (tid & 31) >> 2, k4 = (tid & 3) * 2;
                for (uint32_t base = (tid >> 5) * GROUPS_PER_WARP; base < P; base += (WC_THREADS / 32) * GROUPS_PER_WARP) {
                    const uint32_t o = base + sub;
                    const bool act = o < P;
                    unsigned int n = 0, nfull = 0, off0 = 0;
                    uint4 keep0 = make_uint4(0, 0, 0, 0), keep1 = keep0;
                    uint4 *src = reinterpret_cast<uint4 *>(s_buf + (act ? o : 0) * row_stride);
                    if (act) {
                        n = min(s_fill[o], row_cap);
                        nfull = n / WC_LINE;
                        off0 = s_off[o];
                        unsigned short *qbase = qset + ((size_t)o * P + p) * cap;
                        keep0 = src[nfull * 8 + k4];
                        keep1 = src[nfull * 8 + k4 + 1];
                        for (unsigned int l = 0; l < nfull; l++) {
                            if (off0 + WC_LINE <= cap) {
                                uint4 *dst = reinterpret_cast<uint4 *>(qbase + off0);
                                const uint4 a0 = src[l * 8 + k4], a1 = src[l * 8 + k4 + 1];
                                dst[k4] = a0;
                                dst[k4 + 1] = a1;
                                off0 += WC_LINE;
                            } else if (k4 == 0) {
                                const unsigned short *r = s_buf + o * row_stride + l * WC_LINE;
                                for (unsigned int k = 0; k < (unsigned int)WC_LINE; k++) wc_spill(r[k], o, P, pc, prm.o);
                            }
                        }
                    }
                    __syncwarp();
                    if (act) {
                        if (nfull) { src[k4] = keep0; src[k4 + 1] = keep1; }
                        if (k4 == 0) { s_off[o] = off0; s_fill[o] = n - nfull * WC_LINE; }
                    }
                }
                __syncthreads();
            }
        };
        for (int part = 0; part < (PAIR ? 2 : 1); part++) {
            const size_t lo = part == 0 ? tile0 : max(tile0, tiles_seg0);
            const size_t hi = part == 0 ? min(tile0 + ntile_all, tiles_seg0) : tile0 + ntile_all;
            if (hi <= lo) continue;
            const uint32_t ntile = (uint32_t)(hi - lo);
            const bool as_i64 = part == 1;
            const size_t first = (part == 0 ? lo : lo - tiles_seg0) * S::TILE + (size_t)tid * 4;
            vptr = reinterpret_cast<const char *>(part == 0 ? prm.vals : prm.vals2) + first * 8;
            iptr = (part == 0 ? ids : reinterpret_cast<const IdT *>(prm.ids2)) + first;
            load_tile(vptr, iptr, cur, cur_id);
            auto prefetch_ahead = [&](uint32_t tile_loaded) {
                if (prm.pf_tiles && tile_loaded + prm.pf_tiles < ntile) {
#pragma unroll
                    for (int g = 0; g < GROUPS; g++) {
                        asm volatile("prefetch.global.L2 [%0];" ::"l"(vptr + pf_v + (size_t)g * WC_THREADS * 32));
                        if ((tid & 3) == 0) asm volatile("prefetch.global.L2 [%0];" ::"l"(iptr + pf_i + (size_t)g * WC_THREADS * 4));
                    }
                }
            };
            for (uint32_t t = 0; t < ntile; t += 2) {
                vptr += (size_t)S::TILE * 8;
                iptr += S::TILE;
                if (t + 1 < ntile) load_tile(vptr, iptr, nxt, nxt_id);
                prefetch_ahead(t + 1);
                bin_tile(cur, cur_id, as_i64);
                if (t + 1 >= ntile) break;
                vptr += (size_t)S::TILE * 8;
                iptr += S::TILE;
                if (t + 2 < ntile) load_tile(vptr, iptr, cur, cur_id);
                prefetch_ahead(t + 2);
                bin_tile(nxt, nxt_id, as_i64);
            }
        }
        __syncthreads();
        {
            const unsigned int nr = min(*s_rare, WC_RARE_CAP);
            for (unsigned int i = tid; i < nr; i += WC_THREADS) {
                const uint4 e = rareq[i];
                ValT r;
                const unsigned long long raw = ((unsigned long long)e.y << 32) | e.x;
                memcpy(&r, &raw, 8);
                keyed_one_direct<ValT>(e.z, r, pc, prm.o);
            }
            __syncthreads();
            if (tid == 0) *s_rare = 0;
        }
        if (last_chunk) {
            if (tid < P) {
                const uint32_t o = tid;
                const unsigned int n = min(s_fill[o], row_cap);
                unsigned int off0 = s_off[o];
                const uint4 *src = reinterpret_cast<const uint4 *>(s_buf + o * row_stride);
                for (unsigned int l = 0; l * WC_LINE < n; l++) {
                    const unsigned int nrec = min((unsigned int)WC_LINE, n - l * WC_LINE);
                    if (off0 + WC_LINE <= cap) {
                        uint4 *dst = reinterpret_cast<uint4 *>(qset + ((size_t)o * P + p) * cap + off0);
#pragma unroll
                        for (int k = 0; k < 8; k++) dst[k] = src[l * 8 + k];
                        off0 += nrec;
                    } else {
                        const unsigned short *r = s_buf + o * row_stride + l * WC_LINE;
                        for (unsigned int k = 0; k < nrec; k++) wc_spill(r[k], o, P, pc, prm.o);
                    }
                }
                s_off[o] = off0;
                s_fill[o] = 0;
            }
            __syncthreads();
        }
        if (tid < P) { cset[(size_t)tid * P + p] = s_off[tid]; }
        grid_barrier(prm.barrier, (unsigned int)((c + 1) * (size_t)P));
        if (tid < P) s_off[tid] = __ldcg(&cset[(size_t)p * P + tid]);
        __syncthreads();
        {
            const unsigned short *qmine = qset + (size_t)p * P * cap;
            const uint32_t lane = tid & 31;
#define LH_WC_INC2(word)                                                                                              \
            asm volatile("red.shared.add.u32 [%0], 1;" ::"r"(hist_addr + (((word) << 2) & 0x3FFFCu)) : "memory");     \
            asm volatile("red.shared.add.u32 [%0], 1;" ::"r"(hist_addr + (((word) >> 14) & 0x3FFFCu)) : "memory");
            for (uint32_t w = tid >> 5; w < P; w += WC_THREADS / 32) {
                const unsigned int cnt = s_off[w];
                const unsigned short *q = qmine + (size_t)w * cap;
                const uint4 *qv = reinterpret_cast<const uint4 *>(q);
                const unsigned int nv = cnt >> 3;
#pragma unroll 2
                for (unsigned int i = lane; i < nv; i += 32) {
                    const uint4 v4 = __ldcg(qv + i);
                    LH_WC_INC2(v4.x) LH_WC_INC2(v4.y) LH_WC_INC2(v4.z) LH_WC_INC2(v4.w)
                }
                const unsigned int r0 = nv * 8u + lane;
                if (r0 < cnt) asm volatile("red.shared.add.u32 [%0], 1;" ::"r"(hist_addr + (unsigned int)__ldcg(q + r0) * 4u) : "memory");
            }
#undef LH_WC_INC2
        }
        __syncthreads();
        if (tid < P) s_off[tid] = 0;
    }
    __syncthreads();
    for (uint32_t lid = 0; lid < prm.ids_per; lid++) {
        const uint32_t id = lid * P + p;
        if (id >= prm.o.H) break;
        int any = 0;
        for (uint32_t slot = tid; slot < pc.win; slot += WC_THREADS) {
            const unsigned int cnt = s_hist[lid * pc.win + slot];
            if (cnt) { atomicAdd(&prm.o.buckets[(size_t)id * 65536u + slot], (unsigned long long)cnt); any = 1; }
        }
        any = __syncthreads_or(any);
        if (any && tid == 0) mark(&prm.o.flags[id], 1u);
    }
}

__global__ void k_fold_hot(unsigned int *__restrict__ hot, unsigned long long *__restrict__ buckets, uint32_t *__restrict__ flags,
                           size_t cells, uint32_t replicas, uint32_t win) {
    const size_t stride = (size_t)gridDim.x * blockDim.x;
    const uint32_t row = 2u * win;
    for (size_t i = (size_t)blockIdx.x * blockDim.x + threadIdx.x; i < cells; i += stride) {
        unsigned long long sum = 0;
        for (uint32_t r = 0; r < replicas; r++) {
            unsigned int *cell = hot + (size_t)r * cells + i;
            if (*cell) sum += atomicExch(cell, 0u);
        }
        if (sum) {
            size_t h = i / row;
            uint32_t slot = (uint32_t)(i - h * row);
            atomicAdd(&buckets[h * 65536u + slot_to_key16(slot, win)], sum);
            mark(&flags[h], 1u);
        }
    }
}

constexpr int K2_SMEM_COUNTERS = 8192;

template <typename IdT, int THREADS>
__global__ void __launch_bounds__(THREADS)
k_counter_add_smem(const IdT *__restrict__ ids, const unsigned long long *__restrict__ amounts, size_t n,
                   unsigned long long *__restrict__ counters, uint32_t C,
                   unsigned long long *__restrict__ dropped) {
    extern __shared__ unsigned int s_cnt[];
    unsigned int *lo = s_cnt, *hi = s_cnt + C;
    for (uint32_t i = threadIdx.x; i < 2 * C; i += THREADS) s_cnt[i] = 0;
    __syncthreads();
    const size_t stride = (size_t)gridDim.x * THREADS;
    for (size_t i = (size_t)blockIdx.x * THREADS + threadIdx.x; i < n; i += stride) {
        uint32_t id = (uint32_t)ids[i];
        unsigned long long amt = amounts[i];
        if (id >= C) { atomicAdd(dropped, 1ull); continue; }
        unsigned int a_lo = (unsigned int)amt, a_hi = (unsigned int)(amt >> 32);
        unsigned int old = atomicAdd(&lo[id], a_lo);
        a_hi += (old + a_lo < old) ? 1u : 0u;
        if (a_hi) atomicAdd(&hi[id], a_hi);
    }
    __syncthreads();
    for (uint32_t i = threadIdx.x; i < C; i += THREADS) {
        unsigned long long v = ((unsigned long long)hi[i] << 32) | lo[i];
        if (v) atomicAdd(&counters[i], v);
    }
}

template <typename IdT, int THREADS>
__global__ void __launch_bounds__(THREADS)
k_counter_add_smem_vec(const IdT *__restrict__ ids, const unsigned long long *__restrict__ amounts, size_t n4,
                       unsigned long long *__restrict__ counters, uint32_t C, unsigned long long *__restrict__ dropped) {
    extern __shared__ unsigned int s_cnt[];
    unsigned int *lo = s_cnt, *hi = s_cnt + C;
    for (uint32_t i = threadIdx.x; i < 2 * C; i += THREADS) s_cnt[i] = 0;
    __syncthreads();
    const size_t stride = (size_t)gridDim.x * THREADS;
    size_t g = (size_t)blockIdx.x * THREADS + threadIdx.x;
    unsigned long long cur[4], nxt[4];
    IdPack<IdT> cid, nid;
    if (g < n4) { load_vals4(amounts, g, cur); cid.load(ids, g); }
    for (; g < n4; g += stride) {
        const size_t gn = g + stride;
        if (gn < n4) { load_vals4(amounts, gn, nxt); nid.load(ids, gn); }
#pragma unroll
        for (int j = 0; j < 4; j++) {
            const uint32_t id = cid.get(j);
            const unsigned long long amt = cur[j];
            if (id >= C) { atomicAdd(dropped, 1ull); continue; }
            const unsigned int a_lo = (unsigned int)amt;
            unsigned int a_hi = (unsigned int)(amt >> 32);
            const unsigned int old = atomicAdd(&lo[id], a_lo);
            a_hi += (old + a_lo < old) ? 1u : 0u;
            if (a_hi) atomicAdd(&hi[id], a_hi);
        }
#pragma unroll
        for (int j = 0; j < 4; j++) cur[j] = nxt[j];
        cid = nid;
    }
    __syncthreads();
    for (uint32_t i = threadIdx.x; i < C; i += THREADS) {
        unsigned long long v = ((unsigned long long)hi[i] << 32) | lo[i];
        if (v) atomicAdd(&counters[i], v);
    }
}

template <typename IdT, int THREADS>
__global__ void __launch_bounds__(THREADS)
k_counter_add(const IdT *__restrict__ ids, const unsigned long long *__restrict__ amounts, size_t n,
              unsigned long long *__restrict__ counters, uint32_t C,
              unsigned long long *__restrict__ dropped) {
    const size_t stride = (size_t)gridDim.x * THREADS;
    for (size_t i = (size_t)blockIdx.x * THREADS + threadIdx.x; i < n; i += stride) {
        uint32_t id = (uint32_t)ids[i];
        if (id < C) atomicAdd(&counters[id], amounts[i]);
        else atomicAdd(dropped, 1ull);
    }
}

__global__ void k_merge_sparse(const uint32_t *__restrict__ ids, const short *__restrict__ keys,
                               const unsigned long long *__restrict__ counts, size_t n, uint32_t H,
                               unsigned long long *__restrict__ buckets, uint32_t *__restrict__ flags,
                               unsigned long long *__restrict__ dropped, uint32_t win) {
    const size_t stride = (size_t)gridDim.x * blockDim.x;
    for (size_t i = (size_t)blockIdx.x * blockDim.x + threadIdx.x; i < n; i += stride) {
        const uint32_t id = ids[i];
        if (id >= H) { atomicAdd(dropped, 1ull); continue; }
        add_bucket_global(buckets + (size_t)id * 65536u, flags + id, (uint32_t)(int)keys[i] & 0xFFFFu, counts[i], win);
    }
}

constexpr int K3_THREADS = 1024;
constexpr int K3_WARP_KEYS = 2048;

__device__ __forceinline__ bool warp_scans(int key0, uint32_t level, uint32_t win) {
    if (level & 2u) return true;
    return key0 <= (int)win - 1 && key0 + K3_WARP_KEYS - 1 >= -((int)win - 1);
}

__device__ __forceinline__ void reduce_dense(uint32_t level, const unsigned long long *__restrict__ buckets, const uint32_t *__restrict__ flags, uint32_t win,
         const double *__restrict__ decomp,
         const double *__restrict__ ps, int np, unsigned long long *__restrict__ out_count,
         double *__restrict__ out_sum, double *__restrict__ out_avg, int *__restrict__ out_pkeys,
         double *__restrict__ out_pvals, uint32_t *__restrict__ out_nnz) {
    __shared__ unsigned long long s_cnt[32];
    __shared__ unsigned long long s_tot[32];
    __shared__ double s_sum[32];
    __shared__ unsigned int s_nnz[32];
    __shared__ int s_owner[LH_MAX_PCT];
    __shared__ unsigned long long s_total;
    const int h = blockIdx.x, t = threadIdx.x, lane = t & 31, warp = t >> 5;
    const unsigned long long *hb = buckets + (size_t)h * 65536u;
    const int key0 = -32768 + warp * K3_WARP_KEYS;
    const bool scans = warp_scans(key0, level, win);

    unsigned long long mine = 0;
    double msum = 0.0;
    unsigned int nnz = 0;
    if (scans) {
#pragma unroll 16
        for (int r = 0; r < K3_WARP_KEYS / 32; r++) {
            unsigned int slot = (unsigned int)(key0 + r * 32 + lane) & 0xFFFFu;
            unsigned long long c = hb[slot];
            if (c) { mine += c; msum += decomp[slot] * (double)c; nnz++; }
        }
    }
#pragma unroll
    for (int o = 16; o > 0; o >>= 1) {
        mine += __shfl_xor_sync(0xFFFFFFFFu, mine, o);
        msum += __shfl_xor_sync(0xFFFFFFFFu, msum, o);
        nnz += __shfl_xor_sync(0xFFFFFFFFu, nnz, o);
    }
    if (lane == 0) { s_cnt[warp] = mine; s_tot[warp] = mine; s_sum[warp] = msum; s_nnz[warp] = nnz; }
    if (t < LH_MAX_PCT) s_owner[t] = 0x7FFFFFFF;
    __syncthreads();
    if (warp == 0) {
        unsigned long long w = s_cnt[lane], wi = w;
#pragma unroll
        for (int o = 1; o < 32; o <<= 1) {
            unsigned long long y = __shfl_up_sync(0xFFFFFFFFu, wi, o);
            if (lane >= o) wi += y;
        }
        s_cnt[lane] = wi - w;
        if (lane == 31) s_total = wi;
        double ts = s_sum[lane];
        unsigned int tn = s_nnz[lane];
#pragma unroll
        for (int o = 16; o > 0; o >>= 1) {
            ts += __shfl_xor_sync(0xFFFFFFFFu, ts, o);
            tn += __shfl_xor_sync(0xFFFFFFFFu, tn, o);
        }
        if (lane == 0) { s_sum[0] = ts; s_nnz[0] = tn; }
    }
    __syncthreads();
    const unsigned long long total = s_total;
    const double ftotal = (double)total;
    if (lane == 0 && s_tot[warp]) {
        const unsigned long long end_incl = s_cnt[warp] + s_tot[warp];
        for (int j = 0; j < np; j++)
            if (__ddiv_rn((double)end_incl, ftotal) >= ps[j]) atomicMin(&s_owner[j], warp);
    }
    __syncthreads();
    unsigned int pending = 0;
    for (int j = 0; j < np; j++) if (s_owner[j] == warp) pending |= 1u << j;
    if (pending) {
        unsigned long long sofar = s_cnt[warp];
        for (int r = 0; r < K3_WARP_KEYS / 32 && pending; r++) {
            int key = key0 + r * 32 + lane;
            unsigned long long c = hb[(unsigned int)key & 0xFFFFu];
            unsigned long long incl = c;
#pragma unroll
            for (int o = 1; o < 32; o <<= 1) {
                unsigned long long y = __shfl_up_sync(0xFFFFFFFFu, incl, o);
                if (lane >= o) incl += y;
            }
            const double frac = __ddiv_rn((double)(sofar + incl), ftotal);
            for (int j = 0; j < np; j++) {
                if (!(pending >> j & 1u)) continue;
                unsigned int hit = __ballot_sync(0xFFFFFFFFu, c != 0 && frac >= ps[j]);
                if (hit) {
                    if (lane == __ffs(hit) - 1) {
                        out_pkeys[(size_t)h * np + j] = key;
                        out_pvals[(size_t)h * np + j] = decomp[(unsigned int)key & 0xFFFFu];
                    }
                    pending &= ~(1u << j);
                }
            }
            sofar += __shfl_sync(0xFFFFFFFFu, incl, 31);
        }
    }
    if (t == 0) {
        for (int j = 0; j < np; j++)
            if (s_owner[j] == 0x7FFFFFFF) {
                out_pkeys[(size_t)h * np + j] = (int)0x80000000;
                out_pvals[(size_t)h * np + j] = __longlong_as_double(0x7FF8000000000000ll);
            }
        out_count[h] = total;
        out_sum[h] = s_sum[0];
        out_avg[h] = __ddiv_rn(s_sum[0], ftotal);
        out_nnz[h] = s_nnz[0];
    }
}

__device__ __forceinline__ bool percentile_threshold(double p, unsigned long long total, unsigned long long *T) {
    const double ft = (double)total;
    if (!(__ddiv_rn(ft, ft) >= p)) return false;
    auto ok = [&](unsigned long long s) { return __ddiv_rn((double)s, ft) >= p; };
    unsigned long long s = 0;
    if (p > 0.0) {
        const double est = ceil(p * ft);
        s = est >= ft ? total : (unsigned long long)est;
    }
    int steps = 0;
    while (s > 0 && ok(s - 1) && steps < 8) { s--; steps++; }
    while (!ok(s) && steps < 16) { s++; steps++; }
    if (steps >= 8 && (!ok(s) || (s > 0 && ok(s - 1)))) {
        unsigned long long lo = 0, hi = total;
        while (lo < hi) { const unsigned long long mid = lo + (hi - lo) / 2; if (ok(mid)) hi = mid; else lo = mid + 1; }
        s = lo;
    }
    *T = s;
    return true;
}

__global__ void __launch_bounds__(K3_THREADS)
k_reduce(const unsigned long long *__restrict__ buckets, const uint32_t *__restrict__ flags, uint32_t win,
         const double *__restrict__ decomp,
         const double *__restrict__ ps, int np, unsigned long long *__restrict__ out_count,
         double *__restrict__ out_sum, double *__restrict__ out_avg, int *__restrict__ out_pkeys,
         double *__restrict__ out_pvals, uint32_t *__restrict__ out_nnz, uint32_t smem_cells) {
    extern __shared__ __align__(16) unsigned long long k3_cells[];
    const int h = blockIdx.x, t = threadIdx.x, lane = t & 31, warp = t >> 5;
    const uint32_t level = flags[h];
    if (level == 0) {
        if (t == 0) {
            out_count[h] = 0; out_sum[h] = 0.0; out_avg[h] = __longlong_as_double(0x7FF8000000000000ll); out_nnz[h] = 0;
            for (int j = 0; j < np; j++) {
                out_pkeys[(size_t)h * np + j] = (int)0x80000000;
                out_pvals[(size_t)h * np + j] = __longlong_as_double(0x7FF8000000000000ll);
            }
        }
        return;
    }
    const uint32_t n = 2u * win - 1u;
    if ((level & 2u) || smem_cells < n) {
        reduce_dense(level, buckets, flags, win, decomp, ps, np, out_count, out_sum, out_avg, out_pkeys, out_pvals, out_nnz);
        return;
    }
    __shared__ unsigned long long s_c[32];
    __shared__ double s_s[32];
    __shared__ unsigned int s_n[32];
    __shared__ unsigned long long s_total;
    const unsigned long long *hb = buckets + (size_t)h * 65536u;
    constexpr int PER = 32;
    unsigned long long mine = 0;
    double msum = 0.0;
    unsigned int nnz = 0;
    for (uint32_t i = t; i < n; i += K3_THREADS) {
        const unsigned int slot = (unsigned int)((int)i - (int)(win - 1u)) & 0xFFFFu;
        const unsigned long long c = hb[slot];
        k3_cells[i] = c;
        if (c) { mine += c; msum += decomp[slot] * (double)c; nnz++; }
    }
#pragma unroll
    for (int o = 16; o > 0; o >>= 1) {
        mine += __shfl_xor_sync(0xFFFFFFFFu, mine, o);
        msum += __shfl_xor_sync(0xFFFFFFFFu, msum, o);
        nnz += __shfl_xor_sync(0xFFFFFFFFu, nnz, o);
    }
    if (lane == 0) { s_c[warp] = mine; s_s[warp] = msum; s_n[warp] = nnz; }
    __syncthreads();
    if (warp == 0) {
        unsigned long long c = s_c[lane];
        double sm = s_s[lane];
        unsigned int nz = s_n[lane];
#pragma unroll
        for (int o = 16; o > 0; o >>= 1) {
// ... 435 lines not shown
```

Baseline: 389.8 billion.

## Add TMA producer-warp ring pipeline and 16-bit shared histogram to keyed WC kernel

Restructures the write-combining keyed ingest kernel so a dedicated producer warp bulk-copies value/id tiles into a multi-stage shared-memory ring guarded by mbarriers, while the remaining warps consume and bin. The L2 prefetch path and its knob go away. The shared histogram is packed to 16-bit cells, with an escape that spills 32768 to global on overflow, freeing shared memory for the ring and larger owner rows. The queue drain is rebalanced into fixed rounds across warps, and the host side now picks an aligned head offset so the kernel also takes unaligned inputs. The cost is extra complexity, a barrier on every stage, and more atomics for overflow handling.

```diff
diff --git a/loghisto_b200/csrc/lh_api.cu b/loghisto_b200/csrc/lh_api.cu
--- a/loghisto_b200/csrc/lh_api.cu
+++ b/loghisto_b200/csrc/lh_api.cu
@@ -163,7 +163,6 @@
     uint32_t hot_replicas = 1;
     int keyed_mode = 0;
     int64_t kp_chunk = 256 << 20;
-    uint32_t wc_pf_tiles = 1;
     uint32_t wc_flush_samples = 24576;
     int wc_spt = 6;
     unsigned short *d_kp_queues = nullptr;
@@ -305,6 +304,13 @@
 uint32_t ks_ids_per_pass(const lh_ctx *ctx) { return std::max<uint32_t>(1, (uint32_t)(KS_SMEM_BYTES / ((size_t)ctx->pc.win * 4))); }
 
 constexpr size_t kSmemBudget = 227 * 1024;
+constexpr size_t kWcRingBytes = 64 * 1024;
+template <typename IdT, typename ValT>
+size_t wc_head(const IdT *ids, const ValT *vals) {
+    for (size_t h = 0; h < 8; h++)
+        if ((((uintptr_t)(ids + h) | (uintptr_t)(vals + h)) & 15u) == 0) return h;
+    return SIZE_MAX;
+}
 template <typename IdT, typename ValT, int SPT>
 lh_status launch_keyed_wc_spt(lh_ctx *ctx, int b, const IdT *ids, const ValT *vals, size_t n4x4, cudaStream_t s, bool *used, size_t *taken,
                               const IdT *ids2 = nullptr, const long long *vals2 = nullptr, size_t n2 = 0, size_t *taken2 = nullptr) {
@@ -315,14 +321,20 @@
     if (P < 8 || n4x4 + n2 == 0) return LH_OK;
     const uint32_t ids_per = (ctx->H + P - 1) / P;
     using S = WcShape<SPT>;
-    const size_t hist_bytes = (((size_t)ids_per * ctx->pc.win + 3) & ~(size_t)3) * 4;
+    constexpr size_t stage_bytes = (size_t)S::STAGE * (8 + sizeof(IdT));
+    const size_t fixed = (size_t)2 * WC_MAX_STAGES * 8 + ((((size_t)ids_per * ctx->pc.win + 1) / 2 + 3) & ~(size_t)3) * 4 +
+                         (size_t)2 * WC_MAX_PARTS * 4;
+    uint32_t stages = (uint32_t)std::min<size_t>(WC_MAX_STAGES, std::max<size_t>(2, (kWcRingBytes + stage_bytes - 1) / stage_bytes));
     uint32_t row_cap = 0;
-    size_t smem = 0;
-    for (uint32_t cap_try : {256u, 192u, 128u}) {
-        smem = hist_bytes + 2 * WC_MAX_PARTS * 4 + (size_t)(P + 1) * (cap_try + WC_ROW_EXTRA) * 2;
-        if (smem <= kSmemBudget) { row_cap = cap_try; break; }
+    for (;; stages--) {
+        const size_t used_bytes = fixed + stages * stage_bytes;
+        const size_t per_owner = used_bytes < kSmemBudget ? (kSmemBudget - used_bytes) / ((size_t)(P + 1) * 2) : 0;
+        const size_t cap_fit = per_owner > (size_t)WC_ROW_EXTRA ? (per_owner - WC_ROW_EXTRA) / WC_LINE * WC_LINE : 0;
+        if (cap_fit >= 2 * WC_LINE) { row_cap = (uint32_t)cap_fit; break; }
+        if (stages == 2) break;
     }
     if (!row_cap || (size_t)ids_per * ctx->pc.win > 65535) return LH_OK;
+    const size_t smem = fixed + stages * stage_bytes + (size_t)(P + 1) * (row_cap + WC_ROW_EXTRA) * 2;
     if (ctx->keyed_mode != 2 && n4x4 + n2 < ((size_t)1 << 22)) return LH_OK;
     n4x4 = n4x4 / S::TILE * S::TILE;
     n2 = n2 / S::TILE * S::TILE;
@@ -356,7 +368,7 @@
     const double m_max = std::pow((-3.5 + std::sqrt(3.5 * 3.5 + 4.0 * room)) / 2.0, 2.0);
     const uint32_t flush_samples = std::min<uint32_t>(ctx->wc_flush_samples, (uint32_t)(m_max * P));
     prm.flush_tiles = std::max<uint32_t>(1u, flush_samples / S::TILE);
-    prm.pf_tiles = ctx->wc_pf_tiles;
+    prm.stages = stages;
     prm.row_cap = row_cap;
     prm.row_stride = row_cap + WC_ROW_EXTRA;
     prm.slice_tiles = (uint32_t)slice_tiles; prm.queues = ctx->d_kp_queues; prm.q_cnt = ctx->d_kp_cnt;
@@ -399,58 +411,57 @@
         size_t m = (size_t)std::min<unsigned long long>(n - done, kCap - ctx->buf[b].hot_pending);
         const IdT *ids = d_ids + done;
         const ValT *vals = d_vals + done;
-        size_t head = std::min<size_t>(m, ((32u - ((uintptr_t)vals & 31u)) & 31u) / 8u);
-        bool vec_ok = (((uintptr_t)(ids + head)) & (4 * sizeof(IdT) - 1)) == 0;
-        size_t n4 = vec_ok ? (m - head) / 4 : 0;
-        size_t tail_off = head + n4 * 4;
-        if (!vec_ok) { head = 0; tail_off = 0; }
-        if (head) {
-            k_ingest_keyed<IdT, ValT, T><<<1, T, 0, s>>>(ids, vals, head, ko, ctx->pc);
+        size_t lo = 0, hi = 0, hot_used = 0;
+        const size_t head = std::min<size_t>(m, ((32u - ((uintptr_t)vals & 31u)) & 31u) / 8u);
+        const bool vec_ok = (((uintptr_t)(ids + head)) & (4 * sizeof(IdT) - 1)) == 0;
+        const size_t n4 = vec_ok ? (m - head) / 4 : 0;
+        bool used = false;
+        constexpr uint32_t KS_MAX_PASSES = 4;
+        const uint32_t per_max = ks_ids_per_pass(ctx);
+        const uint32_t passes = (ctx->H + per_max - 1) / per_max;
+        if (passes <= KS_MAX_PASSES && ctx->keyed_mode == 0 && n4 >= 4096) {
+            const uint32_t per = (ctx->H + passes - 1) / passes;
+            const size_t smem = ((size_t)per * ctx->pc.win + 4) * 4;
+            const void *fn = (const void *)k_ingest_keyed_small<IdT, ValT>;
+            LH_CUDA(ctx, cudaFuncSetAttribute(fn, cudaFuncAttributeMaxDynamicSharedMemorySize, (int)smem));
+            int grid = (int)std::max<size_t>(1, std::min<size_t>((size_t)(ctx->sm_count - ctx->k1_reserve_sms),
+                                                                  n4 / (KS_THREADS * 16)));
+            for (uint32_t id_lo = 0; id_lo < ctx->H; id_lo += per) {
+                const uint32_t cnt = std::min(per, ctx->H - id_lo);
+                k_ingest_keyed_small<IdT, ValT><<<grid, KS_THREADS, smem, s>>>(ids + head, vals + head, n4, id_lo, cnt, ko, ctx->pc);
+                ctx->stats.kernel_launches++;
+            }
+            used = true;
+            lo = head; hi = head + n4 * 4;
+            hot_used = n4 * 4;
+            ctx->keyed_kernel = "k_ingest_keyed_small";
+        }
+        const size_t wh = wc_head(ids, vals);
+        if (!used && ctx->keyed_mode != 1 && wh < m) {
+            size_t taken = 0;
+            st = launch_keyed_wc<IdT, ValT>(ctx, b, ids + wh, vals + wh, m - wh, s, &used, &taken);
+            if (st != LH_OK) return st;
+            if (used) {
+                ctx->keyed_kernel = "k_ingest_keyed_wc";
+                lo = wh; hi = wh + taken;
+            }
+        }
+        if (!used && n4) {
+            int grid = grid_1d(ctx, n4, T, 1, ctx->keyed_blocks_per_sm);
+            k_ingest_keyed_vec<IdT, ValT, T><<<grid, T, 0, s>>>(ids + head, vals + head, n4, ctx->hot_replicas, ko, ctx->pc);
+            ctx->stats.kernel_launches++;
+            lo = head; hi = head + n4 * 4;
+            hot_used = n4 * 4;
+            ctx->keyed_kernel = "k_ingest_keyed_vec";
+        }
+        if (lo) {
+            k_ingest_keyed<IdT, ValT, T><<<1, T, 0, s>>>(ids, vals, lo, ko, ctx->pc);
             ctx->stats.kernel_launches++;
         }
-        size_t hot_used = 0;
-        if (n4) {
-            bool used = false;
-            constexpr uint32_t KS_MAX_PASSES = 4;
-            const uint32_t per_max = ks_ids_per_pass(ctx);
-            const uint32_t passes = (ctx->H + per_max - 1) / per_max;
-            if (passes <= KS_MAX_PASSES && ctx->keyed_mode == 0 && n4 >= 4096) {
-                const uint32_t per = (ctx->H + passes - 1) / passes;
-                const size_t smem = ((size_t)per * ctx->pc.win + 4) * 4;
-                const void *fn = (const void *)k_ingest_keyed_small<IdT, ValT>;
-                LH_CUDA(ctx, cudaFuncSetAttribute(fn, cudaFuncAttributeMaxDynamicSharedMemorySize, (int)smem));
-                int grid = (int)std::max<size_t>(1, std::min<size_t>((size_t)(ctx->sm_count - ctx->k1_reserve_sms),
-                                                                      n4 / (KS_THREADS * 16)));
-                for (uint32_t lo = 0; lo < ctx->H; lo += per) {
-                    const uint32_t cnt = std::min(per, ctx->H - lo);
-                    k_ingest_keyed_small<IdT, ValT><<<grid, KS_THREADS, smem, s>>>(ids + head, vals + head, n4, lo, cnt, ko, ctx->pc);
-                    ctx->stats.kernel_launches++;
-                }
-                used = true;
-                hot_used = n4 * 4;
-                ctx->keyed_kernel = "k_ingest_keyed_small";
-            }
-            if (!used && ctx->keyed_mode != 1) {
-                size_t taken = 0;
-                st = launch_keyed_wc<IdT, ValT>(ctx, b, ids + head, vals + head, n4 * 4, s, &used, &taken);
-                if (st != LH_OK) return st;
-                if (used) {
-                    ctx->keyed_kernel = "k_ingest_keyed_wc";
-                    tail_off = head + taken;
-                }
-            }
-            if (!used) {
-                int grid = grid_1d(ctx, n4, T, 1, ctx->keyed_blocks_per_sm);
-                k_ingest_keyed_vec<IdT, ValT, T><<<grid, T, 0, s>>>(ids + head, vals + head, n4, ctx->hot_replicas, ko, ctx->pc);
-                ctx->stats.kernel_launches++;
-                hot_used = n4 * 4;
-                ctx->keyed_kernel = "k_ingest_keyed_vec";
-            }
-        }
-        if (tail_off < m) {
-            size_t r = m - tail_off;
+        if (hi < m) {
+            size_t r = m - hi;
             int grid = grid_1d(ctx, r, T, 1, ctx->keyed_blocks_per_sm);
-            k_ingest_keyed<IdT, ValT, T><<<grid, T, 0, s>>>(ids + tail_off, vals + tail_off, r, ko, ctx->pc);
+            k_ingest_keyed<IdT, ValT, T><<<grid, T, 0, s>>>(ids + hi, vals + hi, r, ko, ctx->pc);
             ctx->stats.kernel_launches++;
         }
         LH_CUDA(ctx, cudaGetLastError());
@@ -466,7 +477,7 @@
 template <typename IdT>
 lh_status launch_keyed_pair(lh_ctx *ctx, const IdT *ids_f, const double *vals_f, size_t n_f, const IdT *ids_ns, const long long *vals_ns,
                             size_t n_ns, cudaStream_t s) {
-    auto aligned = [](const void *v, const void *i) { return (((uintptr_t)v & 31u) == 0) && (((uintptr_t)i & (4 * sizeof(IdT) - 1)) == 0); };
+    auto aligned = [](const void *v, const void *i) { return (((uintptr_t)v | (uintptr_t)i) & 15u) == 0; };
     const uint32_t small_passes = (ctx->H + ks_ids_per_pass(ctx) - 1) / ks_ids_per_pass(ctx);
     const bool small = small_passes <= 4 && ctx->keyed_mode == 0;
     const bool fuse = n_f && n_ns && ctx->keyed_mode != 1 && !small && aligned(vals_f, ids_f) && aligned(vals_ns, ids_ns);
@@ -1710,11 +1721,6 @@
         ctx->keyed_mode = (int)value;
         return LH_OK;
     }
-    if (!strcmp(key, "wc_pf")) {
-        if (value < 0 || value > 8) return fail(ctx, LH_ERR_RANGE, "wc_pf is 0 ... 8 tiles");
-        ctx->wc_pf_tiles = (uint32_t)value;
-        return LH_OK;
-    }
     if (!strcmp(key, "wc_flush")) {
         if (value < 4096 || value > 65536) return fail(ctx, LH_ERR_RANGE, "wc_flush is 4096 ... 65536 samples");
         ctx->wc_flush_samples = (uint32_t)value;
diff --git a/loghisto_b200/csrc/lh_kernels.cuh b/loghisto_b200/csrc/lh_kernels.cuh
--- a/loghisto_b200/csrc/lh_kernels.cuh
+++ b/loghisto_b200/csrc/lh_kernels.cuh
@@ -387,6 +387,9 @@
     __device__ __forceinline__ void load(const unsigned short *ids, size_t g) {
         asm volatile("ld.global.nc.L1::no_allocate.v2.u32 {%0, %1}, [%2];" : "=r"(lo), "=r"(hi) : "l"(reinterpret_cast<const char *>(ids) + g * 8));
     }
+    __device__ __forceinline__ void from_stage(const void *stage_ids, uint32_t t, int half) {
+        (half ? hi : lo) = reinterpret_cast<const unsigned int *>(stage_ids)[t];
+    }
     __device__ __forceinline__ uint32_t get(int j) const { const unsigned int w = j < 2 ? lo : hi; return (j & 1) ? (w >> 16) : (w & 0xFFFFu); }
 };
 template <> struct IdPack<unsigned int> {
@@ -394,6 +397,10 @@
     __device__ __forceinline__ void load(const unsigned int *ids, size_t g) {
         asm volatile("ld.global.nc.L1::no_allocate.v4.u32 {%0, %1, %2, %3}, [%4];" : "=r"(w[0]), "=r"(w[1]), "=r"(w[2]), "=r"(w[3])
                      : "l"(reinterpret_cast<const char *>(ids) + g * 16));
+    }
+    __device__ __forceinline__ void from_stage(const void *stage_ids, uint32_t t, int half) {
+        const uint2 x = reinterpret_cast<const uint2 *>(stage_ids)[t];
+        w[2 * half] = x.x; w[2 * half + 1] = x.y;
     }
     __device__ __forceinline__ uint32_t get(int j) const { return w[j]; }
 };
@@ -494,13 +501,20 @@
 
 constexpr int WC_MAX_PARTS = 160;
 constexpr int WC_LINE = 64;
+constexpr int WC_MAX_STAGES = 8;
 
 template <int SPT> struct WcShape {
     static constexpr int THREADS = SPT == 4 ? 1024 : SPT == 6 ? 896 : SPT == 3 ? 768 : 512;
+    static constexpr int CT = THREADS - 32;
     static constexpr int PER = SPT == 8 ? 8 : 4;
-    static constexpr int TILE = THREADS * PER;
+    static constexpr int TILE = CT * PER;
+    static constexpr int STAGE = CT * 2;
+    static constexpr int TILE_STAGES = PER / 2;
 };
 constexpr int WC_ROW_EXTRA = WC_LINE + 8;
+constexpr uint32_t WC_ROUND_VECS = 4;
+constexpr uint32_t WC_ROUND_RECORDS = WC_ROUND_VECS * 8;
+static_assert(1024u * WC_ROUND_RECORDS <= 0x8000u, "one round must not carry a 16-bit window cell past 0xFFFF");
 
 struct WcParams {
     const void *ids;
@@ -514,7 +528,7 @@
     uint32_t slice_tiles;
     uint32_t inv_p;
     uint32_t flush_tiles;
-    uint32_t pf_tiles;
+    uint32_t stages;
     uint32_t row_cap;
     uint32_t row_stride;
     unsigned short *queues;
@@ -525,8 +539,17 @@
 };
 constexpr uint32_t WC_RARE_CAP = 8192;
 
+template <int NT> __device__ __forceinline__ void bar_consumers() { asm volatile("bar.sync 1, %0;" ::"n"(NT) : "memory"); }
+template <int NT> __device__ __forceinline__ bool bar_consumers_or(bool v) {
+    uint32_t r;
+    asm volatile("{\n\t.reg .pred p, q;\n\tsetp.ne.u32 q, %1, 0;\n\tbar.red.or.pred p, 1, %2, q;\n\tselp.u32 %0, 1, 0, p;\n\t}"
+                 : "=r"(r) : "r"((uint32_t)v), "n"(NT) : "memory");
+    return r != 0;
+}
+
+template <int NT>
 __device__ __forceinline__ void grid_barrier(unsigned int *bar, unsigned int target) {
-    __syncthreads();
+    bar_consumers<NT>();
     if (threadIdx.x == 0) {
         __threadfence();
         atomicAdd(bar, 1u);
@@ -535,12 +558,13 @@
             asm volatile("ld.acquire.gpu.global.u32 %0, [%1];" : "=r"(v) : "l"(bar) : "memory");
         } while (v < target);
     }
-    __syncthreads();
-}
-
-__device__ __forceinline__ void wc_spill(uint32_t rec, uint32_t owner, uint32_t P, const Prec &pc, const KeyedOut &o) {
+    bar_consumers<NT>();
+}
+
+__device__ __forceinline__ void wc_spill(uint32_t rec, uint32_t owner, uint32_t P, const Prec &pc, const KeyedOut &o,
+                                         unsigned long long c = 1ull) {
     const uint32_t lid = rec / pc.win, slot = rec - lid * pc.win, id = lid * P + owner;
-    add_bucket_global(o.buckets + (size_t)id * 65536u, o.flags + id, slot, 1ull, pc.win);
+    add_bucket_global(o.buckets + (size_t)id * 65536u, o.flags + id, slot, c, pc.win);
 }
 
 template <typename IdT, typename ValT, int SPT, bool PAIR = false>
@@ -548,12 +572,18 @@
 k_ingest_keyed_wc(WcParams prm, Prec pc) {
     static_assert(!PAIR || std::is_same<ValT, double>::value, "the int64 segment rides on the float64 instantiation");
     using S = WcShape<SPT>;
-    constexpr int WC_THREADS = S::THREADS;
+    constexpr int CT = S::CT;
     constexpr int GROUPS = S::PER / 4;
-    extern __shared__ __align__(16) unsigned char wc_smem[];
+    constexpr uint32_t STAGE_BYTES = S::STAGE * (8u + (uint32_t)sizeof(IdT));
+    static_assert(STAGE_BYTES % 128 == 0 && (S::STAGE * 8) % 16 == 0, "bulk copies need 16-byte sizes and addresses");
+    extern __shared__ __align__(128) unsigned char wc_smem[];
     const uint32_t P = gridDim.x, p = blockIdx.x, tid = threadIdx.x;
-    unsigned int *s_hist = reinterpret_cast<unsigned int *>(wc_smem);
-    const uint32_t hist_words = prm.ids_per * pc.win;
+    const uint32_t stages = prm.stages;
+    unsigned char *ring = wc_smem;
+    uint64_t *full = reinterpret_cast<uint64_t *>(wc_smem + (size_t)stages * STAGE_BYTES);
+    uint64_t *empty = full + WC_MAX_STAGES;
+    unsigned int *s_hist = reinterpret_cast<unsigned int *>(empty + WC_MAX_STAGES);
+    const uint32_t hist_words = (prm.ids_per * pc.win + 1u) / 2u;
     unsigned int *s_fill = s_hist + ((hist_words + 3u) & ~3u);
     unsigned int *s_off = s_fill + WC_MAX_PARTS;
     unsigned short *s_buf = reinterpret_cast<unsigned short *>(s_off + WC_MAX_PARTS);
@@ -566,228 +596,258 @@
     uint32_t negP = 0u - P;
     asm volatile("mov.b32 %0, %0;" : "+r"(negP));
 
-    for (uint32_t i = tid; i < hist_words; i += WC_THREADS) s_hist[i] = 0;
+    for (uint32_t i = tid; i < hist_words; i += S::THREADS) s_hist[i] = 0;
     if (tid < WC_MAX_PARTS) { s_fill[tid] = 0; s_off[tid] = 0; }
-    uint32_t one_bits;
-    asm volatile("mov.b32 %0, 0x3F800000;" : "=r"(one_bits));
+    if (tid == 0) {
+        for (uint32_t s = 0; s < stages; s++) { mbar_init(&full[s], 1); mbar_init(&empty[s], CT / 32); }
+        asm volatile("fence.mbarrier_init.release.cluster;" ::: "memory");
+    }
     __syncthreads();
 
     const size_t tiles_seg0 = prm.n / S::TILE;
     const size_t tiles_total = tiles_seg0 + (PAIR ? prm.n2 / S::TILE : 0);
     const size_t chunk_tiles = (size_t)prm.slice_tiles * P;
     const size_t nchunks = (tiles_total + chunk_tiles - 1) / chunk_tiles;
-    const IdT *ids = reinterpret_cast<const IdT *>(prm.ids);
-    const unsigned int cap = prm.cap;
-    const uint32_t row_cap = prm.row_cap, row_stride = prm.row_stride;
-
-
-    unsigned long long cur[GROUPS][4], nxt[GROUPS][4];
-    IdPack<IdT> cur_id[GROUPS], nxt_id[GROUPS];
-    uint32_t since_flush = 0;
-    const char *vptr = nullptr;
-    const IdT *iptr = nullptr;
-    const size_t pf_v = (size_t)prm.pf_tiles * S::TILE * 8, pf_i = (size_t)prm.pf_tiles * S::TILE;
-    auto load_tile = [&](const char *vp, const IdT *ip, unsigned long long (&raw)[GROUPS][4], IdPack<IdT> (&idp)[GROUPS]) {
-#pragma unroll
-        for (int g = 0; g < GROUPS; g++) {
-            load_vals4(vp, (size_t)g * WC_THREADS, raw[g]);
-            idp[g].load(ip, (size_t)g * WC_THREADS);
-        }
-    };
-
-    for (size_t c = 0; c < nchunks; c++) {
-        const size_t par = c & 1;
-        unsigned short *qset = prm.queues + par * (size_t)P * P * cap;
-        unsigned int *cset = prm.q_cnt + par * (size_t)P * P;
-        const bool last_chunk = c + 1 == nchunks;
-        const size_t tile0 = c * chunk_tiles + (size_t)p * prm.slice_tiles;
-        const uint32_t ntile_all = tile0 >= tiles_total ? 0u : (uint32_t)min((size_t)prm.slice_tiles, tiles_total - tile0);
-        auto bin_tile = [&](unsigned long long (&raw)[GROUPS][4], IdPack<IdT> (&idp)[GROUPS], const bool as_i64) {
-            if constexpr (PAIR) {
-                if (as_i64) {
-#pragma unroll
-                    for (int g = 0; g < GROUPS; g++)
-#pragma unroll
-                        for (int j = 0; j < 4; j++) raw[g][j] = (unsigned long long)__double_as_longlong(__ll2double_rn((long long)raw[g][j]));
+
+    if (tid >= CT) {
+        if (tid == CT) {
+            const uint64_t pol = policy_evict_first();
+            uint32_t s = 0, ph = 0;
+            for (size_t c = 0; c < nchunks; c++) {
+                const size_t t0 = c * chunk_tiles + (size_t)p * prm.slice_tiles;
+                const size_t t1 = min(t0 + prm.slice_tiles, tiles_total);
+                for (size_t t = t0; t < t1; t++) {
+                    const bool i64 = PAIR && t >= tiles_seg0;
+                    const size_t first = (i64 ? t - tiles_seg0 : t) * S::TILE;
+                    const char *vsrc = reinterpret_cast<const char *>(i64 ? prm.vals2 : prm.vals) + first * 8;
+                    const IdT *isrc = reinterpret_cast<const IdT *>(i64 ? prm.ids2 : prm.ids) + first;
+                    for (int k = 0; k < S::TILE_STAGES; k++) {
+                        mbar_wait(&empty[s], ph ^ 1);
+                        unsigned char *dst = ring + s * STAGE_BYTES;
+                        mbar_expect_tx(&full[s], STAGE_BYTES);
+                        bulk_g2s(dst, vsrc + (size_t)k * S::STAGE * 8, S::STAGE * 8, &full[s], pol);
+                        bulk_g2s(dst + S::STAGE * 8, isrc + (size_t)k * S::STAGE, S::STAGE * (uint32_t)sizeof(IdT), &full[s], pol);
+                        if (++s == stages) { s = 0; ph ^= 1; }
+                    }
                 }
             }
-#pragma unroll
-            for (int g = 0; g < GROUPS; g++) {
-                double v[4];
-#pragma unroll
-                for (int j = 0; j < 4; j++) { ValT r; memcpy(&r, &raw[g][j], 8); v[j] = sample_to_f64<ValT>(r); }
-                uint32_t idx[4];
-                bool flag[4];
-                bucket_offsets_v2<4, false, 0>(v, pc, one_bits, idx, flag);
-                bool any = false;
-#pragma unroll
-                for (int j = 0; j < 4; j++) {
-                    const uint32_t id = idp[g].get(j);
-                    const uint32_t lid = __umulhi(id, prm.inv_p), owner = lid * negP + id;
-                    const uint32_t rec = lid * pc.win + idx[j];
-                    const bool rare = flag[j] | (id >= prm.o.H);
-                    const uint32_t oe = rare ? P : owner;
-                    uint32_t pos;
-                    asm volatile("atom.shared.add.u32 %0, [%1], 1;" : "=r"(pos) : "r"(fill_addr + oe * 4u) : "memory");
-                    flag[j] = rare | (pos >= row_cap);
-                    if (!flag[j])
-                        asm volatile("st.shared.u16 [%0], %1;" ::"r"(buf_addr + (oe * row_stride + pos) * 2u), "h"((unsigned short)rec) : "memory");
-                    any |= flag[j];
+        }
+    } else {
+        const unsigned int cap = prm.cap;
+        const uint32_t row_cap = prm.row_cap, row_stride = prm.row_stride;
+        uint32_t one_bits;
+        asm volatile("mov.b32 %0, 0x3F800000;" : "=r"(one_bits));
+        uint32_t since_flush = 0;
+        uint32_t rs = 0, rph = 0;
+        auto take_stage = [&](unsigned long long (&raw)[4], IdPack<IdT> &idp, int half) {
+            mbar_wait(&full[rs], rph);
+            const unsigned char *st = ring + rs * STAGE_BYTES;
+            const ulonglong2 d = reinterpret_cast<const ulonglong2 *>(st)[tid];
+            raw[2 * half] = d.x;
+            raw[2 * half + 1] = d.y;
+            idp.from_stage(st + S::STAGE * 8, tid, half);
+            __syncwarp();
+            if ((tid & 31) == 0) mbar_arrive(&empty[rs]);
+            if (++rs == stages) { rs = 0; rph ^= 1; }
+        };
+
+        for (size_t c = 0; c < nchunks; c++) {
+            const size_t par = c & 1;
+            unsigned short *qset = prm.queues + par * (size_t)P * P * cap;
+            unsigned int *cset = prm.q_cnt + par * (size_t)P * P;
+            const bool last_chunk = c + 1 == nchunks;
+            const size_t t0 = c * chunk_tiles + (size_t)p * prm.slice_tiles;
+            const size_t t1 = min(t0 + prm.slice_tiles, tiles_total);
+            for (size_t t = t0; t < t1; t++) {
+                unsigned long long raw[GROUPS][4];
+                IdPack<IdT> idp[GROUPS];
+#pragma unroll
+                for (int g = 0; g < GROUPS; g++) { take_stage(raw[g], idp[g], 0); take_stage(raw[g], idp[g], 1); }
+                if constexpr (PAIR) {
+                    if (t >= tiles_seg0) {
+#pragma unroll
+                        for (int g = 0; g < GROUPS; g++)
+#pragma unroll
+                            for (int j = 0; j < 4; j++) raw[g][j] = (unsigned long long)__double_as_longlong(__ll2double_rn((long long)raw[g][j]));
+                    }
                 }
-                if (__any_sync(0xFFFFFFFFu, any)) {
-#pragma unroll
-                    for (int j = 0; j < 4; j++)
-                        if (flag[j]) {
-                            const unsigned int at = atomicAdd(s_rare, 1u);
-                            if (at < WC_RARE_CAP) rareq[at] = make_uint4((unsigned int)raw[g][j], (unsigned int)(raw[g][j] >> 32), idp[g].get(j), 0u);
-                            else keyed_one_slow<ValT>(idp[g].get(j), raw[g][j], pc, prm.o);
-                        }
+#pragma unroll
+                for (int g = 0; g < GROUPS; g++) {
+                    double v[4];
+#pragma unroll
+                    for (int j = 0; j < 4; j++) { ValT r; memcpy(&r, &raw[g][j], 8); v[j] = sample_to_f64<ValT>(r); }
+                    uint32_t idx[4];
+                    bool flag[4];
+                    bucket_offsets_v2<4, false, 0>(v, pc, one_bits, idx, flag);
+                    bool any = false;
+#pragma unroll
+                    for (int j = 0; j < 4; j++) {
+                        const uint32_t id = idp[g].get(j);
+                        const uint32_t lid = __umulhi(id, prm.inv_p), owner = lid * negP + id;
+                        const uint32_t rec = lid * pc.win + idx[j];
+                        const bool rare = flag[j] | (id >= prm.o.H);
+                        const uint32_t oe = rare ? P : owner;
+                        uint32_t pos;
+                        asm volatile("atom.shared.add.u32 %0, [%1], 1;" : "=r"(pos) : "r"(fill_addr + oe * 4u) : "memory");
+                        flag[j] = rare | (pos >= row_cap);
+                        if (!flag[j])
+                            asm volatile("st.shared.u16 [%0], %1;" ::"r"(buf_addr + (oe * row_stride + pos) * 2u), "h"((unsigned short)rec) : "memory");
+                        any |= flag[j];
+                    }
+                    if (__any_sync(0xFFFFFFFFu, any)) {
+#pragma unroll
+                        for (int j = 0; j < 4; j++)
+                            if (flag[j]) {
+                                const unsigned int at = atomicAdd(s_rare, 1u);
+                                if (at < WC_RARE_CAP) rareq[at] = make_uint4((unsigned int)raw[g][j], (unsigned int)(raw[g][j] >> 32), idp[g].get(j), 0u);
+                                else keyed_one_slow<ValT>(idp[g].get(j), raw[g][j], pc, prm.o);
+                            }
+                    }
                 }
-            }
-            if (++since_flush == prm.flush_tiles) {
-                since_flush = 0;
-                __syncthreads();
-                constexpr uint32_t GROUPS_PER_WARP = 8;
-                const uint32_t sub = (tid & 31) >> 2, k4 = (tid & 3) * 2;
-                for (uint32_t base = (tid >> 5) * GROUPS_PER_WARP; base < P; base += (WC_THREADS / 32) * GROUPS_PER_WARP) {
-                    const uint32_t o = base + sub;
-                    const bool act = o < P;
-                    unsigned int n = 0, nfull = 0, off0 = 0;
-                    uint4 keep0 = make_uint4(0, 0, 0, 0), keep1 = keep0;
-                    uint4 *src = reinterpret_cast<uint4 *>(s_buf + (act ? o : 0) * row_stride);
-                    if (act) {
-                        n = min(s_fill[o], row_cap);
-                        nfull = n / WC_LINE;
-                        off0 = s_off[o];
-                        unsigned short *qbase = qset + ((size_t)o * P + p) * cap;
-                        keep0 = src[nfull * 8 + k4];
-                        keep1 = src[nfull * 8 + k4 + 1];
-                        for (unsigned int l = 0; l < nfull; l++) {
-                            if (off0 + WC_LINE <= cap) {
-                                uint4 *dst = reinterpret_cast<uint4 *>(qbase + off0);
-                                const uint4 a0 = src[l * 8 + k4], a1 = src[l * 8 + k4 + 1];
-                                dst[k4] = a0;
-                                dst[k4 + 1] = a1;
-                                off0 += WC_LINE;
-                            } else if (k4 == 0) {
-                                const unsigned short *r = s_buf + o * row_stride + l * WC_LINE;
-                                for (unsigned int k = 0; k < (unsigned int)WC_LINE; k++) wc_spill(r[k], o, P, pc, prm.o);
+                if (++since_flush == prm.flush_tiles) {
+                    since_flush = 0;
+                    bar_consumers<CT>();
+                    constexpr uint32_t GROUPS_PER_WARP = 8;
+                    const uint32_t sub = (tid & 31) >> 2, k4 = (tid & 3) * 2;
+                    for (uint32_t base = (tid >> 5) * GROUPS_PER_WARP; base < P; base += (CT / 32) * GROUPS_PER_WARP) {
+                        const uint32_t o = base + sub;
+                        const bool act = o < P;
+                        unsigned int n = 0, nfull = 0, off0 = 0;
+                        uint4 keep0 = make_uint4(0, 0, 0, 0), keep1 = keep0;
+                        uint4 *src = reinterpret_cast<uint4 *>(s_buf + (act ? o : 0) * row_stride);
+                        if (act) {
+                            n = min(s_fill[o], row_cap);
+                            nfull = n / WC_LINE;
+                            off0 = s_off[o];
+                            unsigned short *qbase = qset + ((size_t)o * P + p) * cap;
+                            keep0 = src[nfull * 8 + k4];
+                            keep1 = src[nfull * 8 + k4 + 1];
+                            for (unsigned int l = 0; l < nfull; l++) {
+                                if (off0 + WC_LINE <= cap) {
+                                    uint4 *dst = reinterpret_cast<uint4 *>(qbase + off0);
+                                    const uint4 a0 = src[l * 8 + k4], a1 = src[l * 8 + k4 + 1];
+                                    dst[k4] = a0;
+                                    dst[k4 + 1] = a1;
+                                    off0 += WC_LINE;
+                                } else if (k4 == 0) {
+                                    const unsigned short *r = s_buf + o * row_stride + l * WC_LINE;
+                                    for (unsigned int k = 0; k < (unsigned int)WC_LINE; k++) wc_spill(r[k], o, P, pc, prm.o);
+                                }
                             }
                         }
+                        __syncwarp();
+                        if (act) {
+                            if (nfull) { src[k4] = keep0; src[k4 + 1] = keep1; }
+                            if (k4 == 0) { s_off[o] = off0; s_fill[o] = n - nfull * WC_LINE; }
+                        }
                     }
-                    __syncwarp();
-                    if (act) {
-                        if (nfull) { src[k4] = keep0; src[k4 + 1] = keep1; }
-                        if (k4 == 0) { s_off[o] = off0; s_fill[o] = n - nfull * WC_LINE; }
+                    bar_consumers<CT>();
+                }
+            }
+            bar_consumers<CT>();
+            {
+                const unsigned int nr = min(*s_rare, WC_RARE_CAP);
+                for (unsigned int i = tid; i < nr; i += CT) {
+                    const uint4 e = rareq[i];
+                    ValT r;
+                    const unsigned long long raw = ((unsigned long long)e.y << 32) | e.x;
+                    memcpy(&r, &raw, 8);
+                    keyed_one_direct<ValT>(e.z, r, pc, prm.o);
+                }
+                bar_consumers<CT>();
+                if (tid == 0) *s_rare = 0;
+            }
+            if (last_chunk) {
+                if (tid < P) {
+                    const uint32_t o = tid;
+                    const unsigned int n = min(s_fill[o], row_cap);
+                    unsigned int off0 = s_off[o];
+                    const uint4 *src = reinterpret_cast<const uint4 *>(s_buf + o * row_stride);
+                    for (unsigned int l = 0; l * WC_LINE < n; l++) {
+                        const unsigned int nrec = min((unsigned int)WC_LINE, n - l * WC_LINE);
+                        if (off0 + WC_LINE <= cap) {
+                            uint4 *dst = reinterpret_cast<uint4 *>(qset + ((size_t)o * P + p) * cap + off0);
+#pragma unroll
+                            for (int k = 0; k < 8; k++) dst[k] = src[l * 8 + k];
+                            off0 += nrec;
+                        } else {
+                            const unsigned short *r = s_buf + o * row_stride + l * WC_LINE;
+                            for (unsigned int k = 0; k < nrec; k++) wc_spill(r[k], o, P, pc, prm.o);
+                        }
                     }
+                    s_off[o] = off0;
+                    s_fill[o] = 0;
                 }
-                __syncthreads();
-            }
-        };
-        for (int part = 0; part < (PAIR ? 2 : 1); part++) {
-            const size_t lo = part == 0 ? tile0 : max(tile0, tiles_seg0);
-            const size_t hi = part == 0 ? min(tile0 + ntile_all, tiles_seg0) : tile0 + ntile_all;
-            if (hi <= lo) continue;
-            const uint32_t ntile = (uint32_t)(hi - lo);
-            const bool as_i64 = part == 1;
-            const size_t first = (part == 0 ? lo : lo - tiles_seg0) * S::TILE + (size_t)tid * 4;
-            vptr = reinterpret_cast<const char *>(part == 0 ? prm.vals : prm.vals2) + first * 8;
-            iptr = (part == 0 ? ids : reinterpret_cast<const IdT *>(prm.ids2)) + first;
-            load_tile(vptr, iptr, cur, cur_id);
-            auto prefetch_ahead = [&](uint32_t tile_loaded) {
-                if (prm.pf_tiles && tile_loaded + prm.pf_tiles < ntile) {
-#pragma unroll
-                    for (int g = 0; g < GROUPS; g++) {
-                        asm volatile("prefetch.global.L2 [%0];" ::"l"(vptr + pf_v + (size_t)g * WC_THREADS * 32));
-                        if ((tid & 3) == 0) asm volatile("prefetch.global.L2 [%0];" ::"l"(iptr + pf_i + (size_t)g * WC_THREADS * 4));
+                bar_consumers<CT>();
+            }
+            if (tid < P) { cset[(size_t)tid * P + p] = s_off[tid]; }
+            grid_barrier<CT>(prm.barrier, (unsigned int)((c + 1) * (size_t)P));
+            if (tid < P) s_off[tid] = __ldcg(&cset[(size_t)p * P + tid]);
+            bar_consumers<CT>();
+            {
+                const unsigned short *qmine = qset + (size_t)p * P * cap;
+                const uint32_t lane = tid & 31;
+                uint32_t w = tid >> 5, i = lane;
+                auto escape = [&](uint32_t rec, uint32_t old) {
+                    const uint32_t sh = (rec & 1u) << 4;
+                    if (((old >> sh) & 0xFFFFu) == 0x7FFFu) {
+                        asm volatile("red.shared.add.u32 [%0], %1;" ::"r"(hist_addr + ((rec << 1) & ~3u)), "r"(0u - (0x8000u << sh)) : "memory");
+                        wc_spill(rec, p, P, pc, prm.o, 32768ull);
                     }
-                }
-            };
-            for (uint32_t t = 0; t < ntile; t += 2) {
-                vptr += (size_t)S::TILE * 8;
-                iptr += S::TILE;
-                if (t + 1 < ntile) load_tile(vptr, iptr, nxt, nxt_id);
-                prefetch_ahead(t + 1);
-                bin_tile(cur, cur_id, as_i64);
-                if (t + 1 >= ntile) break;
-                vptr += (size_t)S::TILE * 8;
-                iptr += S::TILE;
-                if (t + 2 < ntile) load_tile(vptr, iptr, cur, cur_id);
-                prefetch_ahead(t + 2);
-                bin_tile(nxt, nxt_id, as_i64);
-            }
-        }
-        __syncthreads();
-        {
-            const unsigned int nr = min(*s_rare, WC_RARE_CAP);
-            for (unsigned int i = tid; i < nr; i += WC_THREADS) {
-                const uint4 e = rareq[i];
-                ValT r;
-                const unsigned long long raw = ((unsigned long long)e.y << 32) | e.x;
-                memcpy(&r, &raw, 8);
-                keyed_one_direct<ValT>(e.z, r, pc, prm.o);
-            }
-            __syncthreads();
-            if (tid == 0) *s_rare = 0;
-        }
-        if (last_chunk) {
-            if (tid < P) {
-                const uint32_t o = tid;
-                const unsigned int n = min(s_fill[o], row_cap);
-                unsigned int off0 = s_off[o];
-                const uint4 *src = reinterpret_cast<const uint4 *>(s_buf + o * row_stride);
-                for (unsigned int l = 0; l * WC_LINE < n; l++) {
-                    const unsigned int nrec = min((unsigned int)WC_LINE, n - l * WC_LINE);
-                    if (off0 + WC_LINE <= cap) {
-                        uint4 *dst = reinterpret_cast<uint4 *>(qset + ((size_t)o * P + p) * cap + off0);
-#pragma unroll
-                        for (int k = 0; k < 8; k++) dst[k] = src[l * 8 + k];
-                        off0 += nrec;
-                    } else {
-                        const unsigned short *r = s_buf + o * row_stride + l * WC_LINE;
-                        for (unsigned int k = 0; k < nrec; k++) wc_spill(r[k], o, P, pc, prm.o);
+                };
+                auto add1 = [&](uint32_t rec) {
+                    uint32_t old;
+                    asm volatile("atom.shared.add.u32 %0, [%1], %2;" : "=r"(old) : "r"(hist_addr + ((rec << 1) & ~3u)), "r"(1u << ((rec & 1u) << 4)) : "memory");
+                    escape(rec, old);
+                };
+                auto add8 = [&](const uint4 &v) {
+                    const uint32_t wd[4] = {v.x, v.y, v.z, v.w};
+                    uint32_t old[8];
+#pragma unroll
+                    for (int j = 0; j < 4; j++) {
+                        asm volatile("atom.shared.add.u32 %0, [%1], %2;" : "=r"(old[2 * j]) : "r"(hist_addr + ((wd[j] << 1) & 0x1FFFCu)), "r"(1u << ((wd[j] & 1u) << 4)) : "memory");
+                        asm volatile("atom.shared.add.u32 %0, [%1], %2;" : "=r"(old[2 * j + 1]) : "r"(hist_addr + ((wd[j] >> 15) & 0x1FFFCu)), "r"(1u << ((wd[j] >> 12) & 16u)) : "memory");
                     }
-                }
-                s_off[o] = off0;
-                s_fill[o] = 0;
-            }
-            __syncthreads();
-        }
-        if (tid < P) { cset[(size_t)tid * P + p] = s_off[tid]; }
-        grid_barrier(prm.barrier, (unsigned int)((c + 1) * (size_t)P));
-        if (tid < P) s_off[tid] = __ldcg(&cset[(size_t)p * P + tid]);
-        __syncthreads();
-        {
-            const unsigned short *qmine = qset + (size_t)p * P * cap;
-            const uint32_t lane = tid & 31;
-#define LH_WC_INC2(word)                                                                                              \
-            asm volatile("red.shared.add.u32 [%0], 1;" ::"r"(hist_addr + (((word) << 2) & 0x3FFFCu)) : "memory");     \
-            asm volatile("red.shared.add.u32 [%0], 1;" ::"r"(hist_addr + (((word) >> 14) & 0x3FFFCu)) : "memory");
-            for (uint32_t w = tid >> 5; w < P; w += WC_THREADS / 32) {
-                const unsigned int cnt = s_off[w];
-                const unsigned short *q = qmine + (size_t)w * cap;
-                const uint4 *qv = reinterpret_cast<const uint4 *>(q);
-                const unsigned int nv = cnt >> 3;
-#pragma unroll 2
-                for (unsigned int i = lane; i < nv; i += 32) {
-                    const uint4 v4 = __ldcg(qv + i);
-                    LH_WC_INC2(v4.x) LH_WC_INC2(v4.y) LH_WC_INC2(v4.z) LH_WC_INC2(v4.w)
-                }
-                const unsigned int r0 = nv * 8u + lane;
-                if (r0 < cnt) asm volatile("red.shared.add.u32 [%0], 1;" ::"r"(hist_addr + (unsigned int)__ldcg(q + r0) * 4u) : "memory");
-            }
-#undef LH_WC_INC2
-        }
-        __syncthreads();
-        if (tid < P) s_off[tid] = 0;
-    }
-    __syncthreads();
+#pragma unroll
+                    for (int j = 0; j < 4; j++) { escape(wd[j] & 0xFFFFu, old[2 * j]); escape(wd[j] >> 16, old[2 * j + 1]); }
+                };
+                do {
+                    uint32_t k = 0;
+                    if (w < P && i + 32u * (WC_ROUND_VECS - 1) < (s_off[w] >> 3)) {
+                        const uint4 *qv = reinterpret_cast<const uint4 *>(qmine + (size_t)w * cap) + i;
+                        uint4 v4[WC_ROUND_VECS];
+#pragma unroll
+                        for (uint32_t u = 0; u < WC_ROUND_VECS; u++) v4[u] = __ldcg(qv + 32u * u);
+#pragma unroll
+                        for (uint32_t u = 0; u < WC_ROUND_VECS; u++) add8(v4[u]);
+                        i += 32u * WC_ROUND_VECS;
+                        k = WC_ROUND_VECS;
+                    }
+                    for (; k < WC_ROUND_VECS && w < P; k++) {
+                        const unsigned int cnt = s_off[w], nv = cnt >> 3;
+                        const unsigned short *q = qmine + (size_t)w * cap;
+                        if (i < nv) {
+                            add8(__ldcg(reinterpret_cast<const uint4 *>(q) + i));
+                            i += 32;
+                        } else {
+                            if (nv * 8u + lane < cnt) add1(__ldcg(q + nv * 8u + lane));
+                            w += CT / 32;
+                            i = lane;
+                        }
+                    }
+                } while (bar_consumers_or<CT>(w < P));
+            }
+            if (tid < P) s_off[tid] = 0;
+        }
+    }
+    __syncthreads();
+    const unsigned short *s_cell = reinterpret_cast<const unsigned short *>(s_hist);
     for (uint32_t lid = 0; lid < prm.ids_per; lid++) {
         const uint32_t id = lid * P + p;
         if (id >= prm.o.H) break;
         int any = 0;
-        for (uint32_t slot = tid; slot < pc.win; slot += WC_THREADS) {
-            const unsigned int cnt = s_hist[lid * pc.win + slot];
+        for (uint32_t slot = tid; slot < pc.win; slot += S::THREADS) {
+            const unsigned int cnt = s_cell[lid * pc.win + slot];
             if (cnt) { atomicAdd(&prm.o.buckets[(size_t)id * 65536u + slot], (unsigned long long)cnt); any = 1; }
         }
         any = __syncthreads_or(any);
```

Measured after the change: 389.6 billion, median of 6. Within noise of the previous version (-0.1%).
